# kmkolasinski/tfrecords-reader

Measured on AMD Instinct MI355X. Metric: GiB/s + examples/s device-resident TFRecord->Feature decode, 1/2/4/8 GPU, higher is better.
Workload: dtype u8; 1 GPU; C4 directory (configs[4]) of 256 files, C1-shaped (int64 label + 12 B bytes_list id) records, 524288 +-50 % per file (default_rng(1000+f)), spec CRC-32C; this rank's LPT share (256 files) resident in HBM; records_per_gpu=134295581, framed_bytes_per_gpu=7906235019, parallelism=file-sharded x1 (LPT by bytes, no collective on the data path), batches_per_gpu=4, batch_bytes_max=1976558779, streams=2, tpl_groups_missed=0

## Files before the change

### include/tfrg.h

```cpp
#ifndef TFRG_H
#define TFRG_H
#include <stdint.h>
#include "tfrg_status.h"

#ifdef __cplusplus
extern "C" {
#endif

#define TFRG_ABI_VERSION 1

#define TFRG_E_ARG (-1)
#define TFRG_E_HIP (-2)
#define TFRG_E_NOMEM (-3)
#define TFRG_E_IO (-4)
#define TFRG_E_LIMIT (-5)

#define TFRG_FLAG_PAYLOAD_ONLY 1u
#define TFRG_FLAG_SPEC_VARINT 2u
#define TFRG_FLAG_NO_CRC 4u
#define TFRG_FLAG_STRICT_CRC 8u
#define TFRG_FLAG_MATERIALIZE_BYTES 16u

int tfrg_abi_version(void);
const char* tfrg_status_exception(int status);
// ... 30 lines not shown
int tfrg_ctx_set_value_caps(tfrg_ctx* ctx, uint64_t int64_values, uint64_t float_values, uint64_t bytes_values);
int tfrg_ctx_device_bytes(tfrg_ctx* ctx, uint64_t* bytes, uint64_t* hint_reruns);
int tfrg_ctx_set_wave_stage(tfrg_ctx* ctx, uint32_t nbytes);
int tfrg_ctx_set_index_chunk(tfrg_ctx* ctx, uint32_t bytes);

#define TFRG_TPL_MAX 32
#define TFRG_TPL_MAX_PAYLOAD 240
#define TFRG_TPL_MAX_ENTRIES 16
#define TFRG_TPL_MAX_SLOTS 16
#define TFRG_TPL_SAMPLE 4096
int tfrg_learn_templates(tfrg_ctx* ctx, const uint8_t* h_bytes, uint64_t nbytes, const uint64_t* h_start,
                         const uint64_t* h_end, uint32_t n, uint32_t flags);
int tfrg_template_count(tfrg_ctx* ctx);
int tfrg_template_frames(tfrg_ctx* ctx);
int tfrg_template_words(tfrg_ctx* ctx, uint32_t* out, uint64_t cap, uint32_t* window_words);
int tfrg_learn_templates_host(uint32_t n_keys, const uint8_t* key_blob, const uint64_t* key_offsets,
                              const uint32_t* key_flags, uint32_t n_slots, const uint32_t* slot_key,
                              const uint8_t* slot_kind, const uint8_t* h_bytes, uint64_t nbytes,
                              const uint64_t* h_start, const uint64_t* h_end, uint32_t n, uint32_t flags,
                              uint32_t* out, uint64_t cap, uint32_t* window_words);
int tfrg_ctx_set_templates(tfrg_ctx* ctx, int on);

int tfrg_ctx_set_profiling(tfrg_ctx* ctx, int on);
int tfrg_profile_last(tfrg_ctx* ctx, float* ms, const char** names, int cap);

int tfrg_set_schema(tfrg_ctx* ctx, uint32_t n_keys, const uint8_t* key_blob, const uint64_t* key_offsets,
                    const uint32_t* key_flags, uint32_t n_slots, const uint32_t* slot_key,
                    const uint8_t* slot_kind);

typedef struct tfrg_host_ctx tfrg_host_ctx;
typedef struct tfrg_host_record {
  int32_t status;
  uint32_t n_entries;
  int64_t aux;
  const uint32_t* key_off;
  const uint32_t* key_len;
  const uint8_t* kind;
  const uint32_t* val_off;
  const uint32_t* val_cnt;
  const int64_t* i64;
  const uint32_t* f32;
  const uint32_t* b_off;
  const uint32_t* b_len;
} tfrg_host_record;
int tfrg_host_ctx_create(tfrg_host_ctx** out);
int tfrg_host_ctx_destroy(tfrg_host_ctx* ctx);
int tfrg_host_decode(tfrg_host_ctx* ctx, const uint8_t* payload, uint64_t len, uint32_t flags, tfrg_host_record* out);

int tfrg_decode_device(tfrg_ctx* ctx, const uint8_t* d_bytes, uint64_t nbytes, const uint64_t* d_start,
                       const uint64_t* d_end, uint32_t n, uint32_t flags, void* stream);
int tfrg_decode_device32(tfrg_ctx* ctx, const uint8_t* d_bytes, uint64_t nbytes, const uint32_t* d_start32,
                         const uint32_t* d_end32, uint32_t first_start, uint32_t n, uint32_t flags, void* stream);
int tfrg_decode_host(tfrg_ctx* ctx, const uint8_t* h_bytes, uint64_t nbytes, const uint64_t* h_start,
                     const uint64_t* h_end, uint32_t n, uint32_t flags, void* stream);

#define TFRG_INDEX_FB_ROUNDS 1u
#define TFRG_INDEX_FB_SEEK 2u
typedef struct tfrg_index_info {
  uint64_t n_records;
  uint32_t fallback;
  uint32_t tiled;
  uint32_t first_start;
  uint32_t n_chunks, repaired_chunks, repair_rounds;
} tfrg_index_info;
int tfrg_index_device(tfrg_ctx* ctx, const uint8_t* d_bytes, uint64_t nbytes, const uint64_t* piece_sizes,
                      uint32_t n_pieces, uint64_t* d_start, uint64_t* d_end, uint32_t* d_end32, uint64_t cap,
                      uint64_t* piece_records, void* stream, tfrg_index_info* info);

typedef struct tfrg_info {
  uint32_t n_records;
  uint32_t n_slots;
  uint32_t n_errors;
  uint32_t first_error;
  uint32_t n_miss_records;
  uint32_t n_miss_entries;
  uint32_t n_big;
  uint32_t scan_timeout;
  uint64_t kind_totals[4];
  uint64_t nbytes;
  uint64_t bytes_data_len;
  uint32_t tpl_groups_missed;
  uint32_t implicit_cols;
  uint64_t placed_slots;
} tfrg_info;

int tfrg_result_info(tfrg_ctx* ctx, tfrg_info* info);

typedef struct tfrg_columns {
  int32_t* status;
  int64_t* aux;
  uint8_t* verdict;
  uint16_t* order;
  uint32_t* row_splits;
  uint64_t* slot_base;
  int64_t* i64;
  uint32_t* f32;
  uint32_t* bytes_off;
  uint32_t* bytes_len;
  uint32_t* miss;
  uint8_t* bytes_data;
  uint64_t* bytes_offsets;
} tfrg_columns;

int tfrg_result_device(tfrg_ctx* ctx, tfrg_columns* cols);
int tfrg_result_fetch(tfrg_ctx* ctx, const tfrg_columns* host);

#define TFRG_DENSE_I64 0
#define TFRG_DENSE_I32 1
#define TFRG_DENSE_F32 2
#define TFRG_DENSE_U8 3
#define TFRG_DENSE_MAX_SPECS 64
#define TFRG_DENSE_MAX_WIDTH 4096
typedef struct tfrg_dense_spec {
  uint32_t slot;
  uint32_t dtype;
  uint32_t width;
  uint32_t reserved;
  uint64_t fill;
  void* out;
  int32_t* lengths;
} tfrg_dense_spec;
int tfrg_result_dense(tfrg_ctx* ctx, const tfrg_dense_spec* specs, uint32_t n_specs, uint32_t* d_stats,
                      void* consumer_stream);

#define TFRG_ROWS_I32 0
#define TFRG_ROWS_I64 1
int tfrg_result_dense_rows(tfrg_ctx* ctx, const tfrg_dense_spec* specs, uint32_t n_specs, const void* d_rows,
                           uint32_t rows_dtype, uint32_t m, int64_t row0, uint32_t* d_stats, uint32_t* d_skipped,
                           void* consumer_stream);

#define TFRG_RAGGED_MAX_SPECS 64
typedef struct tfrg_ragged_spec {
  uint32_t slot;
  uint32_t dtype;
  uint32_t max_len;
  uint32_t reserved;
  uint64_t cap;
  void* values;
  int64_t* offsets;
} tfrg_ragged_spec;
int tfrg_result_ragged_rows(tfrg_ctx* ctx, const tfrg_ragged_spec* specs, uint32_t n_specs,
                            const void* d_rows, uint32_t rows_dtype, uint32_t m, int64_t row0,
                            uint64_t* d_totals, uint32_t* d_stats, void* consumer_stream);
int tfrg_ctx_set_ragged_tile(tfrg_ctx* ctx, uint32_t rows);

#define TFRG_SEL_MAX_TERMS 32
#define TFRG_SEL_VALUE 0
#define TFRG_SEL_ANY 1
#define TFRG_SEL_COUNT 2
#define TFRG_SEL_BYTES_LEN 3
#define TFRG_SEL_STATUS 4
#define TFRG_SEL_EQ 0
#define TFRG_SEL_NE 1
#define TFRG_SEL_LT 2
#define TFRG_SEL_LE 3
#define TFRG_SEL_GT 4
#define TFRG_SEL_GE 5
typedef struct tfrg_select_term {
  uint32_t slot;
  uint32_t subject;
  uint32_t op;
  uint32_t group;
  uint32_t index;
  uint32_t reserved;
  uint64_t operand;
} tfrg_select_term;
#define TFRG_SEL_APPEND 1u
// ... 28 lines not shown
```

### tfrecords-reader_amd/csrc/tfrg_capi.cpp

```cpp
#include <hip/hip_runtime.h>
#include <stdlib.h>
#include <string.h>

#include <algorithm>
#include <map>
#include <numeric>
#include <string>
#include <unordered_map>
#include <vector>

#include "../../include/tfrg.h"
#include "crc32c.h"
#include "tfrg_dense.h"
#include "tfrg_ragged.h"
#include "tfrg_select.h"
#include "tfrg_frame.h"
#include "tfrg_internal.h"
#include "tfrg_learn.h"

namespace tfrg {
void set_error(const std::string& s);

#define HIP_TRY(expr)                                                              \
  do {                                                                             \
// ... 36 lines not shown

}

using namespace tfrg;

struct Offsets {
  const uint64_t* s64 = nullptr;
  const uint64_t* e64 = nullptr;
  const uint32_t* s32 = nullptr;
  const uint32_t* e32 = nullptr;
  uint32_t first = 0;
  uint32_t mode = kOffU64;
};

struct tfrg_ctx {
  int device = 0;
  hipStream_t own_stream = nullptr;
  hipStream_t last_stream = nullptr;
  uint32_t lane_max = 2048;
  uint32_t wave_stage = 0xffffffffu;
  uint64_t record_bound = 0;
  uint64_t call_bound = 0;
  int num_cus = 256;
  uint32_t cu_lds = 65536;
  int tpl_stage = 1;
  uint32_t tpl_gpw = 0;
  DBuf crc_tab, consts;
  DBuf ht, key_hash, key_off, key_blob, key_slot, slot_kind, key_w, krec;
  uint32_t n_keys = 0, n_slots = 0, ht_mask = 0;
  DBuf in_bytes, in_start, in_end;
  DBuf status, aux, verdict, order, count, loc, rs, slot_base, totals, kind_totals;
  DBuf ident;
  size_t ident_n = 0;
  DBuf i64, f32, b_off, b_len, big_list, slow_list, miss, info, tsum, crc_rec, crc_base, crc_part;
  DBuf dq, dq_cnt;
  DBuf lmask, rlist;
  DBuf bdata, boff64, blb, bbig;
  bool materialized = false;
  bool tsum_dirty = true;
  uint32_t info_slot = 0;
  bool info_clean = false;
  uint32_t n = 0;
  uint64_t cap_hint = 0;
  hipEvent_t order_ev = nullptr;
  hipEvent_t consumer_ev[2] = {nullptr, nullptr};
  int dense_nt = 0;
  uint64_t nbytes = 0;
  uint64_t cap_i64 = 0, cap_f32 = 0, cap_b = 0;
  bool have_result = false;
  bool rs_complete = false;
  std::unordered_map<std::string, uint32_t> key_id;
  std::vector<int32_t> key_slot_h;
  DBuf tpl;
  uint32_t n_tpl = 0;
  uint32_t tpl_w = 0;
  size_t tpl_img_off = 0;
  uint32_t tpl_img_words = 0;
  uint32_t tpl_tab_words = 0;
  std::vector<uint32_t> tpl_h;
  bool tpl_learned = false;
  bool tpl_full = false;
  uint32_t tpl_frames = 0;
  bool tpl_on = true;
  std::vector<uint8_t> slot_kind_h;
  DBuf spec;
  std::vector<uint32_t> spec_h;
  bool have_spec = false;
  bool spec_on = true;
  bool profiling = false;
  bool have_events = false;
  hipEvent_t ev[kNumStages + 1] = {};
  uint64_t hint_i64 = 0, hint_f32 = 0, hint_b = 0;
  bool hinted = false;
  bool no_hints = false;
  uint64_t hint_reruns = 0;
  bool optimistic_on = true;
  bool walk_beside = true;
  uint32_t walk_blocks = 0;
  bool no_quiet = false;
  bool opt_pending = false;
  bool ord_const = false;
  bool len_const = false;
  std::vector<uint32_t> const_len;
  uint32_t last_implicit = 0;
  bool last_aux_zero = false;
  uint32_t* info_pin = nullptr;
  bool cols_complete = false;
  bool mat_pending = false;
  struct LastCall {
    const uint8_t* d_bytes;
    uint64_t nbytes;
    uint64_t cap_in;
    uint64_t bound;
    uint32_t n, flags;
    hipStream_t st;
  } last{};
  Offsets last_off{};
  uint32_t index_chunk = kIndexChunkDefault;
  DBuf fr_tab, fr_dev;
  uint32_t ragged_tile = kRaggedTileDefault;
  DBuf rg_tsum;
  uint32_t select_tile = kSelTileDefault;
  DBuf sel_buf;
  void* fr_pin = nullptr;
  size_t fr_pin_cap = 0;
  uint32_t poison[4] = {0xffffffffu, 0xffffffffu, 0xffffffffu, 0xffffffffu};
};

extern "C" {

int tfrg_ctx_create(int device, tfrg_ctx** out) {
  *out = nullptr;
  int ndev = 0;
  HIP_TRY(hipGetDeviceCount(&ndev));
  if (device < 0 || device >= ndev) {
    set_error("bad device index");
    return TFRG_E_ARG;
  }
  HIP_TRY(hipSetDevice(device));
  tfrg_ctx* c = new tfrg_ctx();
  c->device = device;
  if (const char* e = getenv("TFRG_TEMPLATES")) c->tpl_on = atoi(e) != 0;
  if (const char* e = getenv("TFRG_SPEC")) c->spec_on = atoi(e) != 0;
  if (const char* e = getenv("TFRG_TPL_STAGE")) c->tpl_stage = atoi(e);
  if (const char* e = getenv("TFRG_TPL_GPW")) {
    const int v = atoi(e);
    if (v == 2 || v == 4 || v == 8) c->tpl_gpw = (uint32_t)v;
  }
  if (const char* e = getenv("TFRG_OPTIMISTIC")) c->optimistic_on = atoi(e) != 0;
  if (const char* e = getenv("TFRG_WALK_BESIDE")) c->walk_beside = atoi(e) != 0;
  if (const char* e = getenv("TFRG_WALK_BLOCKS")) c->walk_blocks = (uint32_t)atoi(e);
  if (const char* e = getenv("TFRG_DENSE_NT")) c->dense_nt = atoi(e) != 0;
  if (const char* e = getenv("TFRG_DEBUG_POISON_LOC")) {
    char* q = const_cast<char*>(e);
    for (int i = 0; i < 4 && *q; ++i) {
      c->poison[i] = (uint32_t)strtoul(q, &q, 10);
      while (*q == ',' || *q == ' ') ++q;
    }
  }
  hipDeviceProp_t prop;
  if (hipGetDeviceProperties(&prop, device) == hipSuccess) {
    c->num_cus = prop.multiProcessorCount;
    if (prop.maxSharedMemoryPerMultiProcessor) c->cu_lds = (uint32_t)prop.maxSharedMemoryPerMultiProcessor;
  }
  if (hipStreamCreateWithFlags(&c->own_stream, hipStreamNonBlocking) != hipSuccess) {
    delete c;
    set_error("hipStreamCreate failed");
    return TFRG_E_HIP;
  }
  if (hipHostMalloc(reinterpret_cast<void**>(&c->info_pin), (kInfoCount + 8) * 4) != hipSuccess) {
    (void)hipStreamDestroy(c->own_stream);
    delete c;
    set_error("hipHostMalloc failed");
    return TFRG_E_NOMEM;
  }
  std::vector<uint32_t> tab(kCrcTabWords), cst(128);
  CrcTables T;
  crc_make_tables(&T);
  memcpy(tab.data(), T.t, 4096);
  uint32_t M[4][256];
  crc_make_mul_tables(gf_xpow8(1024), M);
  memcpy(tab.data() + 1024, M, 4096);
  memcpy(tab.data() + 2048, T.t, 8192);
  memcpy(tab.data() + 4096, T.t, 16384);
  for (int e = 0; e < 256; ++e)
    for (int col = 0; col < 47; ++col) tab[8192 + e * 64 + col] = T.t[(col + 1) & 15][e];
  crc_make_mul_tables(gf_xpow8(2048), M);
  memcpy(tab.data() + 24576, M, 4096);
  crc_make_mul_tables(gf_xpow8(4096), M);
  memcpy(tab.data() + 25600, M, 4096);
  for (int k = 0; k < 24; ++k) {
    crc_make_mul_tables(gf_xpow8(1024ull << k), M);
    memcpy(tab.data() + 26624 + k * 1024, M, 4096);
  }
  for (int l = 0; l < 64; ++l) cst[l] = gf_xpow8(16ull * l);
  for (int z = 0; z < 16; ++z) cst[64 + z] = gf_xpow8_inv((uint64_t)z);
  for (int k = 0; k < 32; ++k) cst[96 + k] = gf_xpow8(1024ull << k);
  if (c->crc_tab.ensure(tab.size() * 4) != hipSuccess || c->consts.ensure(cst.size() * 4) != hipSuccess ||
      hipMemcpy(c->crc_tab.p, tab.data(), tab.size() * 4, hipMemcpyHostToDevice) != hipSuccess ||
      hipMemcpy(c->consts.p, cst.data(), cst.size() * 4, hipMemcpyHostToDevice) != hipSuccess) {
    set_error("constant upload failed");
    tfrg_ctx_destroy(c);
    return TFRG_E_HIP;
  }
  *out = c;
  return 0;
}

int tfrg_ctx_destroy(tfrg_ctx* c) {
  if (!c) return 0;
  (void)hipSetDevice(c->device);
  if (c->last_stream) (void)hipStreamSynchronize(c->last_stream);
  DBuf* all[] = {&c->crc_tab, &c->consts, &c->ht, &c->key_hash, &c->key_off, &c->key_blob, &c->key_slot,
                 &c->slot_kind, &c->key_w, &c->krec, &c->in_bytes, &c->in_start, &c->in_end, &c->status, &c->aux, &c->verdict,
                 &c->order, &c->count, &c->loc, &c->rs, &c->ident, &c->slot_base, &c->totals, &c->kind_totals, &c->i64,
                 &c->f32, &c->b_off, &c->b_len, &c->big_list, &c->slow_list, &c->miss, &c->info, &c->tsum,
                 &c->bdata, &c->boff64, &c->blb, &c->bbig, &c->crc_rec, &c->crc_base, &c->crc_part, &c->tpl, &c->spec,
                 &c->dq, &c->dq_cnt, &c->lmask, &c->rlist, &c->fr_tab, &c->fr_dev, &c->rg_tsum, &c->sel_buf};
  for (DBuf* b : all) b->release();
  if (c->order_ev) (void)hipEventDestroy(c->order_ev);
  for (hipEvent_t e : c->consumer_ev)
    if (e) (void)hipEventDestroy(e);
  if (c->have_events)
    for (auto& e : c->ev) (void)hipEventDestroy(e);
  if (c->own_stream) (void)hipStreamDestroy(c->own_stream);
  if (c->info_pin) (void)hipHostFree(c->info_pin);
  if (c->fr_pin) (void)hipHostFree(c->fr_pin);
  delete c;
  return 0;
}

int tfrg_ctx_set_lane_max(tfrg_ctx* c, uint32_t lane_max) {
// ... 167 lines not shown
}

static void key_words(const uint8_t* p, uint64_t n, uint32_t* w0, uint32_t* w1) {
  uint32_t a = 0, b = 0;
  for (uint64_t i = 0; i < (n < 4 ? n : 4); ++i) a |= (uint32_t)p[i] << (8 * i);
  if (n > 4)
    for (uint64_t i = 0; i < 4; ++i) b |= (uint32_t)p[n - 4 + i] << (8 * i);
  *w0 = a;
  *w1 = b;
}

int tfrg_set_schema(tfrg_ctx* c, uint32_t n_keys, const uint8_t* key_blob, const uint64_t* key_offsets,
                    const uint32_t* key_flags, uint32_t n_slots, const uint32_t* slot_key, const uint8_t* slot_kind) {
  if (!c) return TFRG_E_ARG;
  HIP_TRY(hipSetDevice(c->device));
  if (c->last_stream) HIP_TRY(hipStreamSynchronize(c->last_stream));
  c->have_result = false;
  c->n_keys = c->n_slots = 0;
  c->ht_mask = 0;
  uint32_t hsz = 16;
  while (hsz < 2 * n_keys + 2) hsz <<= 1;
  std::vector<uint32_t> ht(hsz, 0), hash(n_keys ? n_keys : 1), off(n_keys + 1), kw(2ull * (n_keys ? n_keys : 1));
  std::vector<int32_t> ks(4ull * (n_keys ? n_keys : 1), -1);
  const uint64_t blob_len = n_keys ? key_offsets[n_keys] : 0;
  for (uint32_t k = 0; k < n_keys; ++k) {
    if (key_offsets[k + 1] < key_offsets[k] || key_offsets[k + 1] > 0xffffffffull) {
      set_error("bad key offsets");
      return TFRG_E_ARG;
    }
    off[k] = (uint32_t)key_offsets[k];
    const uint64_t kl = key_offsets[k + 1] - key_offsets[k];
    key_words(key_blob + key_offsets[k], kl, &kw[2ull * k], &kw[2ull * k + 1]);
    hash[k] = key_hash_words((uint32_t)kl, kw[2ull * k], kw[2ull * k + 1]);
    ks[4ull * k] = (int32_t)(key_flags ? (key_flags[k] & 1u) : 0u);
    uint32_t j = hash[k] & (hsz - 1);
    while (ht[j]) j = (j + 1) & (hsz - 1);
    ht[j] = k + 1;
  }
  off[n_keys] = (uint32_t)blob_len;
  for (uint32_t s = 0; s < n_slots; ++s) {
    if (slot_key[s] >= n_keys || slot_kind[s] < 1 || slot_kind[s] > 3) {
      set_error("bad slot");
      return TFRG_E_ARG;
    }
    ks[4ull * slot_key[s] + slot_kind[s]] = (int32_t)s;
  }
  if (c->ht.ensure(hsz * 4) || c->key_hash.ensure(hash.size() * 4) || c->key_off.ensure(off.size() * 4) ||
      c->key_blob.ensure(blob_len + 16) || c->key_slot.ensure(ks.size() * 4) || c->slot_kind.ensure(n_slots + 16) ||
      c->key_w.ensure(kw.size() * 4)) {
    set_error("schema allocation failed");
    return TFRG_E_NOMEM;
  }
  HIP_TRY(hipMemcpy(c->ht.p, ht.data(), hsz * 4, hipMemcpyHostToDevice));
  HIP_TRY(hipMemcpy(c->key_hash.p, hash.data(), hash.size() * 4, hipMemcpyHostToDevice));
  HIP_TRY(hipMemcpy(c->key_off.p, off.data(), off.size() * 4, hipMemcpyHostToDevice));
  if (blob_len) HIP_TRY(hipMemcpy(c->key_blob.p, key_blob, blob_len, hipMemcpyHostToDevice));
  HIP_TRY(hipMemcpy(c->key_slot.p, ks.data(), ks.size() * 4, hipMemcpyHostToDevice));
  HIP_TRY(hipMemcpy(c->key_w.p, kw.data(), kw.size() * 4, hipMemcpyHostToDevice));
  std::vector<uint32_t> kr((size_t)kKrWords * (n_keys ? n_keys : 1), 0);
  for (uint32_t k = 0; k < n_keys; ++k) {
    uint32_t* r = &kr[(size_t)kKrWords * k];
    r[kKrHash] = hash[k];
    r[kKrLen] = (uint32_t)(key_offsets[k + 1] - key_offsets[k]);
    r[kKrW0] = kw[2ull * k];
    r[kKrW1] = kw[2ull * k + 1];
    for (int kind = 1; kind <= 3; ++kind) r[kKrSlot1 + kind - 1] = (uint32_t)ks[4ull * k + kind];
    r[kKrFlags] = (uint32_t)ks[4ull * k];
  }
  if (c->krec.ensure(kr.size() * 4)) {
    set_error("schema allocation failed");
    return TFRG_E_NOMEM;
  }
  HIP_TRY(hipMemcpy(c->krec.p, kr.data(), kr.size() * 4, hipMemcpyHostToDevice));
  if (n_slots) HIP_TRY(hipMemcpy(c->slot_kind.p, slot_kind, n_slots, hipMemcpyHostToDevice));
  c->n_keys = n_keys;
  c->n_slots = n_slots;
  c->ht_mask = hsz - 1;
  c->key_id.clear();
  for (uint32_t k = 0; k < n_keys; ++k)
    c->key_id.emplace(std::string((const char*)key_blob + key_offsets[k], key_offsets[k + 1] - key_offsets[k]), k);
  c->key_slot_h = ks;
  c->slot_kind_h.assign(slot_kind, slot_kind + n_slots);
  c->n_tpl = 0;
  c->tpl_learned = false;
  c->have_spec = false;
  return 0;
}

static DevSchema schema_view(const tfrg_ctx* c) {
  DevSchema s;
  s.n_keys = c->n_keys;
  s.n_slots = c->n_slots;
  s.ht_mask = c->ht_mask;
  s.ht = c->ht.as<uint32_t>();
  s.key_hash = c->key_hash.as<uint32_t>();
  s.key_off = c->key_off.as<uint32_t>();
  s.key_blob = c->key_blob.as<uint8_t>();
  s.key_slot = c->key_slot.as<int32_t>();
  s.slot_kind = c->slot_kind.as<uint8_t>();
  s.key_w = c->key_w.as<uint32_t>();
  s.krec = c->krec.as<uint32_t>();
  s.tpl = c->tpl.as<uint32_t>();
  s.tpl_img = s.tpl + c->tpl_img_off;
  s.tpl_img_words = c->tpl_img_words;
  s.tpl_tab_words = c->tpl_tab_words;
  s.n_tpl = c->tpl_on ? c->n_tpl : 0u;
  s.tpl_w = c->tpl_w;
  s.spec = c->spec_on && c->have_spec ? c->spec.as<uint32_t>() : nullptr;
  return s;
}

extern "C" int tfrg_learn_templates(tfrg_ctx* c, const uint8_t* h_bytes, uint64_t nbytes, const uint64_t* h_start,
                                    const uint64_t* h_end, uint32_t n, uint32_t flags) {
  if (!c || (n && (!h_bytes || !h_start || !h_end))) return TFRG_E_ARG;
  c->tpl_learned = true;
  c->n_tpl = 0;
  c->tpl_frames = 0;
  c->have_spec = false;
  if (!c->n_keys) return 0;
  const TplSchema sch{c->key_id, c->key_slot_h, c->slot_kind_h};
  Learned L;
  const uint32_t nt = learn_shapes(&sch, c->n_slots, h_bytes, nbytes, h_start, h_end, n, flags, L);
  if (!nt && !(L.have_spec = learn_single_slots(&sch, c->n_slots, h_bytes, nbytes, h_start, h_end, n, flags, L.spec)))
    return 0;
  const size_t spec_bytes = (size_t)c->n_slots * 4;
  HIP_TRY(hipSetDevice(c->device));
  if (c->last_stream) HIP_TRY(hipStreamSynchronize(c->last_stream));
  if ((nt && c->tpl.ensure((L.w.size() + L.img.size() + L.ptab.size()) * 4)) ||
      (L.have_spec && c->spec.ensure(spec_bytes))) {
    set_error("template allocation failed");
    return TFRG_E_NOMEM;
  }
  if (nt) {
    uint32_t* const d = c->tpl.as<uint32_t>();
    HIP_TRY(hipMemcpy(d, L.w.data(), L.w.size() * 4, hipMemcpyHostToDevice));
    HIP_TRY(hipMemcpy(d + L.w.size(), L.img.data(), L.img.size() * 4, hipMemcpyHostToDevice));
    if (!L.ptab.empty())
      HIP_TRY(hipMemcpy(d + L.w.size() + L.img.size(), L.ptab.data(), L.ptab.size() * 4, hipMemcpyHostToDevice));
    c->tpl_img_off = L.w.size();
    c->tpl_img_words = (uint32_t)L.img.size();
    c->tpl_tab_words = (uint32_t)L.ptab.size();
    c->n_tpl = nt;
    c->tpl_w = L.W;
    c->tpl_h = L.w;
    c->tpl_full = L.full;
    c->tpl_frames = L.frames;
    c->ord_const = L.ord_const;
    c->len_const = L.len_const;
    c->const_len = L.const_len;
  }
  if (L.have_spec) HIP_TRY(hipMemcpy(c->spec.p, L.spec.data(), spec_bytes, hipMemcpyHostToDevice));
  c->spec_h = L.spec;
  c->have_spec = L.have_spec;
  return (int)nt;
}

extern "C" int tfrg_template_count(tfrg_ctx* c) { return c ? (int)c->n_tpl : TFRG_E_ARG; }

extern "C" int tfrg_template_frames(tfrg_ctx* c) { return c ? (int)(c->n_tpl ? c->tpl_frames : 0u) : TFRG_E_ARG; }

extern "C" int tfrg_template_words(tfrg_ctx* c, uint32_t* out, uint64_t cap, uint32_t* window_words) {
  if (!c) return TFRG_E_ARG;
  if (window_words) *window_words = c->tpl_w;
  const uint64_t nw = (uint64_t)c->n_tpl * kLtWords;
  if (out) memcpy(out, c->tpl_h.data(), (nw < cap ? nw : cap) * 4);
  return (int)c->n_tpl;
}

extern "C" int tfrg_ctx_set_templates(tfrg_ctx* c, int on) {
  if (!c) return TFRG_E_ARG;
  c->tpl_on = on != 0;
  return 0;
}

static int decode_device_any(tfrg_ctx* c, const uint8_t* d_bytes, uint64_t nbytes, const Offsets& off, uint32_t n,
                             uint32_t flags, void* stream);

int tfrg_decode_device(tfrg_ctx* c, const uint8_t* d_bytes, uint64_t nbytes, const uint64_t* d_start,
                       const uint64_t* d_end, uint32_t n, uint32_t flags, void* stream) {
  Offsets off;
  off.s64 = d_start;
  off.e64 = d_end;
  return decode_device_any(c, d_bytes, nbytes, off, n, flags, stream);
}

int tfrg_decode_device32(tfrg_ctx* c, const uint8_t* d_bytes, uint64_t nbytes, const uint32_t* d_start32,
                         const uint32_t* d_end32, uint32_t first_start, uint32_t n, uint32_t flags, void* stream) {
  if (n && !d_end32) return TFRG_E_ARG;
  Offsets off;
  off.s32 = d_start32;
  off.e32 = d_end32;
  off.first = first_start;
  off.mode = d_start32 ? kOffU32 : kOffEnds;
  return decode_device_any(c, d_bytes, nbytes, off, n, flags, stream);
}

static hipError_t launch_materialize_last(tfrg_ctx* c, const uint8_t* d_bytes, uint64_t nbytes, uint64_t cap_in,
                                          uint64_t cap_b, hipStream_t st) {
  uint32_t* const info = c->info.as<uint32_t>() + c->info_slot * kInfoCount;
  DevBytes d;
  d.in = d_bytes;
  d.in_readable = (nbytes + 15) & ~15ull;
  d.b_off = c->b_off.as<uint32_t>();
  d.b_len = c->b_len.as<uint32_t>();
  d.kind_totals = c->kind_totals.as<uint64_t>();
  d.offsets = c->boff64.as<uint64_t>();
  d.offsets_cap = cap_b;
  d.data = c->bdata.as<uint8_t>();
  d.data_cap = cap_in + 16;
  d.lb = c->blb.as<uint64_t>();
  d.ticket = info + kInfoBytesTicket;
  d.big_count = info + kInfoBytesBig;
  d.big_list = c->bbig.as<uint32_t>();
  d.overflow = info + kInfoOverflow;
  return launch_materialize(d, c->num_cus, st);
}

static int decode_device_any(tfrg_ctx* c, const uint8_t* d_bytes, uint64_t nbytes, const Offsets& off, uint32_t n,
                             uint32_t flags, void* stream) {
  if (!c) return TFRG_E_ARG;
  if (nbytes >= (1ull << 32)) {
    set_error("batch larger than 4 GiB: split it");
    return TFRG_E_LIMIT;
  }
  if (c->n_keys == 0) {
    uint64_t z = 0;
    int st = tfrg_set_schema(c, 0, nullptr, &z, nullptr, 0, nullptr, nullptr);
    if (st) return st;
  }
  HIP_TRY(hipSetDevice(c->device));
  c->have_result = false;
  hipStream_t st = stream ? (hipStream_t)stream : c->own_stream;
// ... 63 lines not shown
                    c->bbig.cap < cap_b * 4;
    if (g2 && c->last_stream) HIP_TRY(hipStreamSynchronize(c->last_stream));
    if (c->bdata.ensure(cap_in + 16) || c->boff64.ensure((cap_b + 1) * 8) || c->blb.ensure(lb_words * 8) ||
        c->bbig.ensure(cap_b * 4)) {
      set_error("device allocation failed (materialized bytes)");
      return TFRG_E_NOMEM;
    }
    HIP_TRY(hipMemsetAsync(c->blb.p, 0, lb_words * 8, st));
    if (!n) HIP_TRY(hipMemsetAsync(c->boff64.p, 0, 8, st));
  }
  if (!S || !n) HIP_TRY(hipMemsetAsync(c->kind_totals.p, 0, 32, st));

  DevBatch b;
  b.bytes = d_bytes;
  b.nbytes = nbytes;
  b.start = off.s64;
  b.end = off.e64;
  b.start32 = off.s32;
  b.end32 = off.e32;
  b.first = off.first;
  b.omode = off.mode;
  b.n = n;
  b.flags = flags;
  DevOut o;
  o.status = c->status.as<int32_t>();
  o.aux = c->aux.as<int64_t>();
  o.verdict = c->verdict.as<uint8_t>();
  o.order = c->order.as<uint16_t>();
  o.count = c->count.as<uint32_t>();
  o.loc = c->loc.as<uint2>();
  o.rs = c->rs.as<uint32_t>();
  o.slot_base = c->slot_base.as<uint64_t>();
  o.totals = c->totals.as<uint32_t>();
  o.kind_totals = c->kind_totals.as<uint64_t>();
  o.i64 = c->i64.as<int64_t>();
  o.f32 = c->f32.as<uint32_t>();
  o.b_off = c->b_off.as<uint32_t>();
  o.b_len = c->b_len.as<uint32_t>();
  o.cap_i64 = cap_i64;
  o.cap_f32 = cap_f32;
  o.cap_b = cap_b;
  o.big_list = c->big_list.as<uint32_t>();
  o.miss = c->miss.as<uint32_t>();
  o.miss_cap = kMissCap;
  o.info = info_cur;
  o.info_next = c->info.as<uint32_t>() + (islot ^ 1u) * kInfoCount;
  o.tsum = c->tsum.as<uint32_t>();
  o.tile_stride = tile_stride;
  o.spine_lb = reinterpret_cast<uint64_t*>(o.tsum + (size_t)S * tile_stride);
  o.n_chunks = n_chunks;
  o.irr = o.tsum + (size_t)S * tile_stride + 2ull * S * n_chunks;
  o.slow_list = c->slow_list.as<uint32_t>();
  o.crc_rec = c->crc_rec.as<uint32_t>();
  o.crc_base = c->crc_base.as<uint64_t>();
  o.crc_part = c->crc_part.as<uint64_t>();
  o.lmask = c->lmask.as<uint64_t>();
  o.rlist = c->rlist.as<uint32_t>();
  LaunchCfg cfg;
  cfg.num_cus = c->num_cus;
  cfg.tpl_cu_lds = c->tpl_stage ? c->cu_lds : 0u;
  cfg.tpl_stage_any = c->tpl_stage == 2;
  cfg.tpl_gpw = c->tpl_gpw;
  cfg.lean = c->tpl_on && c->n_tpl;
  cfg.tpl_full = cfg.lean && c->tpl_full;
  cfg.tpl_unchecked = cfg.lean && (c->tpl_frames & 2u) != 0;
  cfg.spec_h = c->spec_h.empty() ? nullptr : c->spec_h.data();
  const uint64_t lane_blocks = (n + 255) / 256;
  const uint64_t lane_cap = (uint64_t)c->num_cus * 8;
  cfg.lane_grid = (int)(lane_blocks < 1 ? 1 : (lane_blocks < lane_cap ? lane_blocks : lane_cap));
  const uint64_t wave_cap = (uint64_t)c->num_cus * 4;
  const uint64_t wave_blocks = (n + 3) / 4;
  cfg.wave_grid = (int)(wave_blocks < 1 ? 1 : (wave_blocks < wave_cap ? wave_blocks : wave_cap));
  cfg.lane_max = c->lane_max;
  cfg.wave_stage = c->wave_stage;
  memcpy(cfg.poison, c->poison, sizeof(cfg.poison));
  cfg.optimistic = c->optimistic_on && !c->no_quiet && c->poison[0] == 0xffffffffu;
  cfg.walk_beside = c->walk_beside;
  cfg.walk_blocks = c->walk_blocks;
  cfg.ran_optimistic = false;
  cfg.ran_quiet_big = false;
  cfg.ord_const = c->ord_const;
  cfg.len_const = c->len_const && !mat;
  cfg.implicit = 0;
  const uint64_t bound = c->call_bound ? c->call_bound : c->record_bound;
  c->call_bound = 0;
  c->last = tfrg_ctx::LastCall{d_bytes, nbytes, cap_in, bound, n, flags, st};
  c->last_off = off;
  o.dq = nullptr;
  o.dq_cnt = nullptr;
  o.dq_blocks = 0;
  cfg.body_count = false;
  if (n && (bound == 0 || bound > c->lane_max)) {
    uint64_t blocks = nbytes >> 18;
    blocks = blocks < 16 ? 16 : (blocks > (1u << 16) ? (1u << 16) : blocks);
    const size_t qb = (size_t)blocks * 64u * kDeferK * 16u, cb = (size_t)blocks * 64u;
    if ((c->dq.cap < qb || c->dq_cnt.cap < cb) && c->last_stream) HIP_TRY(hipStreamSynchronize(c->last_stream));
    if (c->dq.ensure(qb) || c->dq_cnt.ensure(cb)) {
      set_error("device allocation failed (deferred bodies)");
      return TFRG_E_NOMEM;
    }
    o.dq = c->dq.as<uint4>();
    o.dq_cnt = c->dq_cnt.as<uint8_t>();
    o.dq_blocks = (uint32_t)blocks;
    cfg.body_count = true;
  }
  if (n) {
    hipEvent_t* ev = nullptr;
    if (c->profiling) {
      if (!c->have_events) {
        for (auto& e : c->ev) HIP_TRY(hipEventCreate(&e));
        c->have_events = true;
      }
      ev = c->ev;
    }
    hipError_t e = launch_decode(b, schema_view(c), o, cfg, c->crc_tab.as<uint32_t>(), c->consts.as<uint32_t>(), st, ev);
    if (e == hipSuccess && mat && S && !cfg.ran_optimistic) {
      e = launch_materialize_last(c, d_bytes, nbytes, cap_in, cap_b, st);
    } else if (e == hipSuccess && mat && !S) {
      e = hipMemsetAsync(c->boff64.p, 0, 8, st);
    }
    if (ev && e == hipSuccess) e = hipEventRecord(ev[kNumStages], st);
    if (e != hipSuccess) {
      c->tsum_dirty = true;
      set_error(std::string("kernel launch: ") + hipGetErrorString(e));
      return TFRG_E_HIP;
    }
  }
  c->info_clean = n != 0;
  c->n = n;
  c->nbytes = nbytes;
  c->cap_i64 = cap_i64;
  c->cap_f32 = cap_f32;
  c->cap_b = cap_b;
  c->last_stream = st;
  c->materialized = mat;
  c->have_result = true;
  c->rs_complete = false;
  c->opt_pending = n != 0 && cfg.ran_optimistic;
  if (n != 0 && cfg.ran_quiet_big) c->tsum_dirty = true;
  c->mat_pending = c->opt_pending && mat && S;
  c->last_implicit = n != 0 ? cfg.implicit : 0u;
  c->last_aux_zero = n != 0 && cfg.ran_optimistic && !cfg.ran_quiet_big && !(cfg.implicit & TFRG_IMPLICIT_STATUS);
  c->cols_complete = false;
  return 0;
}

int tfrg_decode_host(tfrg_ctx* c, const uint8_t* h_bytes, uint64_t nbytes, const uint64_t* h_start,
                     const uint64_t* h_end, uint32_t n, uint32_t flags, void* stream) {
  if (!c) return TFRG_E_ARG;
  HIP_TRY(hipSetDevice(c->device));
  hipStream_t st = stream ? (hipStream_t)stream : c->own_stream;
  const uint64_t pad = ((nbytes + 15) & ~15ull) + 16;
  if (c->last_stream) HIP_TRY(hipStreamSynchronize(c->last_stream));
  if (c->in_bytes.ensure(pad) || c->in_start.ensure((uint64_t)(n ? n : 1) * 8) ||
      c->in_end.ensure((uint64_t)(n ? n : 1) * 8)) {
    set_error("staging allocation failed");
    return TFRG_E_NOMEM;
  }
  if (nbytes) HIP_TRY(hipMemcpyAsync(c->in_bytes.p, h_bytes, nbytes, hipMemcpyHostToDevice, st));
  HIP_TRY(hipMemsetAsync(c->in_bytes.as<uint8_t>() + nbytes, 0, pad - nbytes, st));
  if (n) {
    HIP_TRY(hipMemcpyAsync(c->in_start.p, h_start, (size_t)n * 8, hipMemcpyHostToDevice, st));
    HIP_TRY(hipMemcpyAsync(c->in_end.p, h_end, (size_t)n * 8, hipMemcpyHostToDevice, st));
  }
  uint64_t total = 0, widest = 0;
  for (uint32_t i = 0; i < n; ++i) {
    const uint64_t a = h_start[i], b = h_end[i] < nbytes ? h_end[i] : nbytes;
    if (b > a) total += b - a;
    if (h_end[i] > a && h_end[i] - a > widest) widest = h_end[i] - a;
  }
  if (!c->tpl_learned && c->n_keys && c->tpl_on) {
    const int t = tfrg_learn_templates(c, h_bytes, nbytes, h_start, h_end, n, flags);
    if (t < 0) return t;
  }
  c->cap_hint = total;
  c->call_bound = widest ? widest : 1;
  return tfrg_decode_device(c, c->in_bytes.as<uint8_t>(), nbytes, c->in_start.as<uint64_t>(),
                            c->in_end.as<uint64_t>(), n, flags, st);
}

static int finish_decode(tfrg_ctx* c, uint32_t* h, uint64_t* kt) {
  bool widened = false;
  for (;;) {
    HIP_TRY(hipMemcpyAsync(c->info_pin, c->info.as<uint32_t>() + c->info_slot * kInfoCount, kInfoCount * 4,
                           hipMemcpyDeviceToHost, c->last_stream));
    HIP_TRY(hipMemcpyAsync(c->info_pin + kInfoCount, c->kind_totals.p, 32, hipMemcpyDeviceToHost, c->last_stream));
    HIP_TRY(hipStreamSynchronize(c->last_stream));
    memcpy(h, c->info_pin, kInfoCount * 4);
    memcpy(kt, c->info_pin + kInfoCount, 32);
    const bool full = c->opt_pending && h[kInfoResid] != 0;
    const bool widen = h[kInfoOverflow] && c->hinted && !widened;
    if (!full && !widen) {
      if (!c->mat_pending) break;
      c->mat_pending = false;
      const tfrg_ctx::LastCall& L = c->last;
      HIP_TRY(launch_materialize_last(c, L.d_bytes, L.nbytes, L.cap_in, c->cap_b, c->last_stream));
      continue;
    }
    const tfrg_ctx::LastCall L = c->last;
    c->no_quiet = true;
    c->no_hints = widen;
    c->cap_hint = L.cap_in;
    c->call_bound = L.bound;
    c->tsum_dirty = true;
    const int rc = decode_device_any(c, L.d_bytes, L.nbytes, c->last_off, L.n, L.flags, L.st);
    c->no_quiet = false;
    c->no_hints = false;
    if (rc) return rc;
    widened |= widen;
    ++c->hint_reruns;
  }
  c->opt_pending = false;
  c->hinted = false;
  return 0;
}

static int overflow_status(const uint32_t* h) {
  if (!h[kInfoOverflow]) return 0;
  set_error("value columns overflowed their capacity (overlapping ranges in a device batch): decode "
            "the ranges from host memory (tfrg_decode_host) or split the batch");
  return TFRG_E_LIMIT;
}

static int confirm_pending(tfrg_ctx* c) {
  if (!c->opt_pending && !c->hinted) return 0;
  HIP_TRY(hipSetDevice(c->device));
  uint32_t h[kInfoCount];
  uint64_t kt[4];
  const int rc = finish_decode(c, h, kt);
  return rc ? rc : overflow_status(h);
}

int tfrg_result_info(tfrg_ctx* c, tfrg_info* info) {
  if (!c || !c->have_result) return TFRG_E_ARG;
  HIP_TRY(hipSetDevice(c->device));
  uint32_t h[kInfoCount] = {0};
  uint64_t kt[4] = {0, 0, 0, 0};
  const int rc = finish_decode(c, h, kt);
  if (rc) return rc;
  uint64_t blen = 0;
  if (c->materialized && !h[kInfoOverflow]) {
    const uint64_t nb = c->n ? kt[TFRG_KIND_BYTES] : 0;
    HIP_TRY(hipMemcpy(&blen, c->boff64.as<uint64_t>() + nb, 8, hipMemcpyDeviceToHost));
  }
  memset(info, 0, sizeof(*info));
  info->n_records = c->n;
  info->n_slots = c->n_slots;
  info->n_errors = h[kInfoErrors];
  info->first_error = ~h[kInfoFirstError];
  info->n_miss_records = h[kInfoMissRecords];
  info->n_miss_entries = h[kInfoMissEntries];
  info->n_big = h[kInfoBigRecs];
  info->scan_timeout = h[kInfoScanTimeout];
  for (int k = 0; k < 4; ++k) info->kind_totals[k] = kt[k];
  info->nbytes = c->nbytes;
  info->bytes_data_len = blen;
  info->tpl_groups_missed = h[kInfoResid];
  info->placed_slots = ((uint64_t)h[kInfoPlacedHi] << 32) | h[kInfoPlacedLo];
  info->implicit_cols = c->last_implicit;
  return overflow_status(h);
}

static std::vector<std::pair<uint64_t, uint32_t>> implicit_len_runs(const tfrg_ctx* c) {
  std::vector<std::pair<uint64_t, uint32_t>> out;
  uint64_t base = 0;
  for (uint32_t k = 0; k < c->n_slots; ++k) {
    if ((c->slot_kind_h[k] & 3u) != TFRG_KIND_BYTES) continue;
    out.push_back({base, k < c->const_len.size() ? c->const_len[k] : 0u});
    base += c->n;
  }
  return out;
}

int tfrg_result_device(tfrg_ctx* c, tfrg_columns* d) {
  if (!c || !c->have_result) return TFRG_E_ARG;
  if (const int rc = confirm_pending(c)) return rc;
  if (!c->rs_complete && c->n_slots && c->n) {
    HIP_TRY(hipSetDevice(c->device));
    HIP_TRY(launch_fill_placed_rows(c->rs.as<uint32_t>(), c->info.as<uint32_t>() + c->info_slot * kInfoCount,
                                    c->n_slots, c->n, c->last_stream));
  }
  c->rs_complete = true;
  if ((c->last_implicit || c->last_aux_zero) && !c->cols_complete) {
    HIP_TRY(hipSetDevice(c->device));
    const size_t n = c->n;
    if (c->last_aux_zero) HIP_TRY(hipMemsetAsync(c->aux.p, 0, n * 8, c->last_stream));
    if (c->last_implicit & TFRG_IMPLICIT_STATUS) {
      HIP_TRY(hipMemsetAsync(c->status.p, 0, n * 4, c->last_stream));
      HIP_TRY(hipMemsetAsync(c->aux.p, 0, n * 8, c->last_stream));
      HIP_TRY(hipMemsetAsync(c->verdict.p, (int)(TFRG_V_LEN_MATCH | TFRG_V_LEN_CRC | TFRG_V_DATA_CRC), n, c->last_stream));
    }
    if (c->last_implicit & TFRG_IMPLICIT_ORDER)
      for (uint32_t k = 0; k < c->n_slots; ++k)
        HIP_TRY(hipMemsetD16Async(reinterpret_cast<hipDeviceptr_t>(c->order.as<uint16_t>() + (size_t)k * n),
                                  (unsigned short)(c->tpl_h[kLtSlot + 3 * k] >> 16), n, c->last_stream));
    if (c->last_implicit & TFRG_IMPLICIT_BYTES_LEN)
      for (const auto& [base, len] : implicit_len_runs(c))
        HIP_TRY(hipMemsetD32Async(reinterpret_cast<hipDeviceptr_t>(c->b_len.as<uint32_t>() + base), (int)len, n,
                                  c->last_stream));
  }
  c->cols_complete = true;
  d->status = c->status.as<int32_t>();
  d->aux = c->aux.as<int64_t>();
  d->verdict = c->verdict.as<uint8_t>();
  d->order = c->order.as<uint16_t>();
  d->row_splits = c->rs.as<uint32_t>();
  d->slot_base = c->slot_base.as<uint64_t>();
  d->i64 = c->i64.as<int64_t>();
  d->f32 = c->f32.as<uint32_t>();
  d->bytes_off = c->b_off.as<uint32_t>();
  d->bytes_len = c->b_len.as<uint32_t>();
  d->miss = c->miss.as<uint32_t>();
  d->bytes_data = c->materialized ? c->bdata.as<uint8_t>() : nullptr;
  d->bytes_offsets = c->materialized ? c->boff64.as<uint64_t>() : nullptr;
  return 0;
}

extern "C++" {
template <class Bad>
static int check_result(const tfrg_ctx* c, const Bad& bad) {
  if (!c) return bad("no context");
  if (!c->have_result) return bad("no result (decode first)");
  return 0;
}
template <class Bad>
static int check_specs(const tfrg_ctx* c, const void* specs, uint32_t n_specs, uint32_t max_specs, const Bad& bad) {
  if (const int rc = check_result(c, bad)) return rc;
  if (!specs || n_specs == 0 || n_specs > max_specs) return bad("n_specs must be 1.." + std::to_string(max_specs));
  return 0;
}
template <class Bad>
static int check_slot_dtype(const tfrg_ctx* c, const std::string& at, uint32_t slot, uint32_t dtype, const Bad& bad) {
  if (slot >= c->n_slots) return bad(at + "slot " + std::to_string(slot) + " >= n_slots");
  const uint32_t kind = c->slot_kind_h[slot] & 3u;
  const bool fits = (kind == TFRG_KIND_INT64 && (dtype == TFRG_DENSE_I64 || dtype == TFRG_DENSE_I32)) ||
                    (kind == TFRG_KIND_FLOAT && dtype == TFRG_DENSE_F32) ||
                    (kind == TFRG_KIND_BYTES && dtype == TFRG_DENSE_U8);
  if (!fits) return bad(at + "dtype " + std::to_string(dtype) + " does not fit the slot's kind " + std::to_string(kind));
  return 0;
}
template <class Bad>
static int check_rows_dtype(const void* d_rows, uint32_t rows_dtype, bool required, const Bad& bad) {
  if ((required || d_rows) && rows_dtype != TFRG_ROWS_I32 && rows_dtype != TFRG_ROWS_I64)
    return bad("rows_dtype must be TFRG_ROWS_I32 or TFRG_ROWS_I64, not " + std::to_string(rows_dtype));
  return 0;
}
template <class Bad>
static int check_rows_m(const void* d_rows, uint32_t m, bool required, const Bad& bad) {
  if (m >= 0x80000000u) return bad("m must be below 2^31");
  if (required && m && !d_rows) return bad("d_rows is NULL");
  return 0;
}

template <class T>
static const T* view_col(const tfrg_ctx* c, const DBuf& b) {
  return static_cast<const T*>(b.p ? b.p : c->slot_base.p);
}
template <class Args>
static void fill_columns(const tfrg_ctx* c, Args& a) {
  a.rs = c->rs.as<uint32_t>();
  a.slot_base = c->slot_base.as<uint64_t>();
  a.i64 = view_col<int64_t>(c, c->i64);
  a.f32 = view_col<uint32_t>(c, c->f32);
  a.b_len = view_col<uint32_t>(c, c->b_len);
  if (c->materialized) a.b_off64 = view_col<uint64_t>(c, c->boff64);
  a.info = c->info.as<uint32_t>() + c->info_slot * kInfoCount;
  a.n = c->n;
}
template <class Args>
static void fill_bytes_source(const tfrg_ctx* c, Args& a) {
  a.b_off = view_col<uint32_t>(c, c->b_off);
  a.in = c->materialized ? c->bdata.as<uint8_t>() : c->last.d_bytes;
  const uint64_t bound = c->materialized ? (uint64_t)c->bdata.cap & ~15ull : (c->last.nbytes + 15ull) & ~15ull;
  a.in_bound = a.in ? (uint32_t)std::min<uint64_t>(bound, 0xfffffff0ull) : 0;
}
}

static_assert(kDenseNoLen == kRaggedNoLen && kRaggedNoLen == kSelNoLen, "one const_len lookup serves all three");
static uint32_t const_len_of(const tfrg_ctx* c, uint32_t slot, bool reads_len) {
  if (!reads_len || !(c->last_implicit & TFRG_IMPLICIT_BYTES_LEN)) return kDenseNoLen;
  return slot < c->const_len.size() ? c->const_len[slot] : 0u;
}

static int fence_open(tfrg_ctx* c, void* consumer_stream, hipStream_t* st, hipStream_t* cs) {
  *st = c->last_stream;
  *cs = consumer_stream ? static_cast<hipStream_t>(consumer_stream) : *st;
  if (*cs == *st) return 0;
  for (hipEvent_t& e : c->consumer_ev)
    if (!e) HIP_TRY(hipEventCreateWithFlags(&e, hipEventDisableTiming));
  HIP_TRY(hipEventRecord(c->consumer_ev[0], *cs));
  HIP_TRY(hipStreamWaitEvent(*st, c->consumer_ev[0], 0));
  return 0;
}
static int fence_close(tfrg_ctx* c, hipStream_t st, hipStream_t cs) {
  if (cs == st) return 0;
  HIP_TRY(hipEventRecord(c->consumer_ev[1], st));
  HIP_TRY(hipStreamWaitEvent(cs, c->consumer_ev[1], 0));
  return 0;
}

struct DenseRows {
  const void* d_rows = nullptr;
  uint32_t dtype = 0, m = 0;
  int64_t row0 = 0;
  uint32_t* d_skipped = nullptr;
};

static int result_dense(const char* fn, bool by_rows, tfrg_ctx* c, const tfrg_dense_spec* specs, uint32_t n_specs,
                        const DenseRows& rows, uint32_t* d_stats, void* consumer_stream) {
  auto bad = [fn](const std::string& why) {
    set_error(std::string(fn) + ": " + why);
    return TFRG_E_ARG;
  };
  if (const int rc = check_specs(c, specs, n_specs, TFRG_DENSE_MAX_SPECS, bad)) return rc;
  static_assert(TFRG_DENSE_MAX_SPECS == kDenseMaxSpecs && TFRG_DENSE_MAX_WIDTH == kDenseMaxWidth &&
                    TFRG_DENSE_I64 == kDenseI64 && TFRG_DENSE_I32 == kDenseI32 && TFRG_DENSE_F32 == kDenseF32 &&
                    TFRG_DENSE_U8 == kDenseU8,
                "tfrg.h mirrors tfrg_dense.h");
  for (uint32_t i = 0; i < n_specs; ++i) {
    const tfrg_dense_spec& s = specs[i];
    const std::string at = "spec " + std::to_string(i) + ": ";
    if (const int rc = check_slot_dtype(c, at, s.slot, s.dtype, bad)) return rc;
    if (s.width == 0 || s.width > TFRG_DENSE_MAX_WIDTH)
      return bad(at + "width must be 1.." + std::to_string(TFRG_DENSE_MAX_WIDTH));
    if (!s.out) return bad(at + "out is NULL");
    if (s.reserved) return bad(at + "reserved must be 0");
  }
  if (by_rows) {
    if (const int rc = check_rows_dtype(rows.d_rows, rows.dtype, true, bad)) return rc;
    if (const int rc = check_rows_m(rows.d_rows, rows.m, true, bad)) return rc;
  }
  if (!by_rows && c->n == 0) return 0;
  HIP_TRY(hipSetDevice(c->device));
  if (const int rc = confirm_pending(c)) return rc;
  const uint32_t out_rows = by_rows ? rows.m : c->n;
  DenseArgs a{};
  if (by_rows) {
    a.rows = rows.d_rows;
    a.rows64 = rows.dtype == TFRG_ROWS_I64;
    a.m = rows.m;
    a.row0 = rows.row0;
    a.skipped = rows.d_skipped;
  }
  fill_columns(c, a);
  fill_bytes_source(c, a);
  a.stats = d_stats;
  a.n_specs = n_specs;
  a.nt = (uint32_t)c->dense_nt;
  const uint64_t cap = std::max<uint64_t>(1, (uint64_t)c->num_cus * 16u / n_specs);
  uint32_t blocks = 0;
  for (uint32_t i = 0; i < n_specs; ++i) {
    const tfrg_dense_spec& s = specs[i];
    DenseSpec& d = a.sp[i];
    d.out = s.out;
    d.lengths = s.lengths;
    d.fill = s.fill;
    d.slot = s.slot;
    d.dtype = s.dtype;
    d.width = s.width;
    d.const_len = const_len_of(c, s.slot, s.dtype == TFRG_DENSE_U8);
    const uint64_t isz = s.dtype == TFRG_DENSE_I64 ? 8 : s.dtype == TFRG_DENSE_U8 ? 1 : 4;
    const uint64_t total = (uint64_t)out_rows * s.width * isz;
    const uint64_t work = ((uintptr_t)s.out & 15u) ? total / isz : (total >> 4) + 16;
    d.blk0 = blocks;
    d.nblk = (uint32_t)std::min<uint64_t>(cap, (work + kDenseChunk - 1) / kDenseChunk);
    blocks += d.nblk;
  }
  hipStream_t st, cs;
  if (const int rc = fence_open(c, consumer_stream, &st, &cs)) return rc;
  const bool one_memset = by_rows && c->n && d_stats && rows.d_skipped == d_stats + 4 * (size_t)n_specs;
  if (d_stats) HIP_TRY(hipMemsetAsync(d_stats, 0, (size_t)n_specs * (one_memset ? 20 : 16), st));
  if (by_rows && rows.d_skipped && !one_memset)
    HIP_TRY(hipMemsetD32Async(reinterpret_cast<hipDeviceptr_t>(rows.d_skipped), c->n ? 0 : (int)rows.m, n_specs, st));
  if (out_rows && c->n) HIP_TRY(launch_dense(a, blocks, st));
  return fence_close(c, st, cs);
}

int tfrg_result_dense(tfrg_ctx* c, const tfrg_dense_spec* specs, uint32_t n_specs, uint32_t* d_stats,
                      void* consumer_stream) {
  return result_dense("tfrg_result_dense", false, c, specs, n_specs, DenseRows{}, d_stats, consumer_stream);
}

int tfrg_result_dense_rows(tfrg_ctx* c, const tfrg_dense_spec* specs, uint32_t n_specs, const void* d_rows,
                           uint32_t rows_dtype, uint32_t m, int64_t row0, uint32_t* d_stats, uint32_t* d_skipped,
                           void* consumer_stream) {
  DenseRows rows;
  rows.d_rows = d_rows;
  rows.dtype = rows_dtype;
  rows.m = m;
  rows.row0 = row0;
  rows.d_skipped = d_skipped;
  return result_dense("tfrg_result_dense_rows", true, c, specs, n_specs, rows, d_stats, consumer_stream);
}

int tfrg_result_ragged_rows(tfrg_ctx* c, const tfrg_ragged_spec* specs, uint32_t n_specs, const void* d_rows,
                            uint32_t rows_dtype, uint32_t m, int64_t row0, uint64_t* d_totals, uint32_t* d_stats,
                            void* consumer_stream) {
  auto bad = [](const std::string& why) {
    set_error("tfrg_result_ragged_rows: " + why);
    return TFRG_E_ARG;
  };
  if (const int rc = check_specs(c, specs, n_specs, TFRG_RAGGED_MAX_SPECS, bad)) return rc;
  static_assert(TFRG_RAGGED_MAX_SPECS == kRaggedMaxSpecs, "tfrg.h mirrors tfrg_ragged.h");
  bool any_values = false;
  for (uint32_t i = 0; i < n_specs; ++i) {
    const tfrg_ragged_spec& s = specs[i];
    const std::string at = "spec " + std::to_string(i) + ": ";
    if (const int rc = check_slot_dtype(c, at, s.slot, s.dtype, bad)) return rc;
    if (!s.offsets) return bad(at + "offsets is NULL");
    if (s.reserved) return bad(at + "reserved must be 0");
    const uintptr_t isz = s.dtype == TFRG_DENSE_I64 ? 8 : s.dtype == TFRG_DENSE_U8 ? 1 : 4;
    if (((uintptr_t)s.values & (isz - 1)) || ((uintptr_t)s.offsets & 7u))
      return bad(at + "values and offsets must be aligned to their element size");
    any_values |= s.values != nullptr && s.cap != 0;
  }
  if (const int rc = check_rows_dtype(d_rows, rows_dtype, false, bad)) return rc;
  if (const int rc = check_rows_m(d_rows, m, false, bad)) return rc;
  const uint32_t tile = c->ragged_tile;
  const uint64_t tiles = ((uint64_t)m + tile - 1) / tile;
  uint64_t split = 1;
  if (any_values && tiles) {
    const uint64_t want = (uint64_t)std::max(c->num_cus, 1) * 4u, have = tiles * n_specs;
    split = std::min<uint64_t>(kRaggedMaxSplit, std::max<uint64_t>(1, (want + have - 1) / have));
  }
  if (tiles * n_specs * split > 0x7fffffffull) return bad("too many tiles for one launch: raise the ragged tile");
  HIP_TRY(hipSetDevice(c->device));
  if (const int rc = confirm_pending(c)) return rc;
  const bool run = m && c->n;
  if (run) HIP_TRY(c->rg_tsum.ensure((size_t)(tiles * n_specs) * 8));
  hipStream_t st, cs;
  if (const int rc = fence_open(c, consumer_stream, &st, &cs)) return rc;
  if (d_stats) HIP_TRY(hipMemsetAsync(d_stats, 0, (size_t)n_specs * 16, st));
  if (run) {
    RaggedArgs a{};
    fill_columns(c, a);
    fill_bytes_source(c, a);
    a.stats = d_stats;
    a.totals = d_totals;
    a.tsum = c->rg_tsum.as<uint64_t>();
    a.rows = d_rows;
    a.rows64 = rows_dtype == TFRG_ROWS_I64;
    a.row0 = row0;
    a.m = m;
    a.n_specs = n_specs;
    a.tile = tile;
    a.tiles = (uint32_t)tiles;
    a.split = (uint32_t)split;
    for (uint32_t i = 0; i < n_specs; ++i) {
      const tfrg_ragged_spec& s = specs[i];
      RaggedSpec& d = a.sp[i];
      d.values = s.values;
      d.offsets = s.offsets;
      d.cap = s.cap;
      d.slot = s.slot;
      d.dtype = s.dtype;
      d.max_len = s.max_len;
      d.const_len = const_len_of(c, s.slot, s.dtype == TFRG_DENSE_U8);
    }
    HIP_TRY(launch_ragged(a, st));
  } else {
    for (uint32_t i = 0; i < n_specs; ++i) {
      HIP_TRY(hipMemsetAsync(specs[i].offsets, 0, ((size_t)m + 1) * 8, st));
      if (d_stats && m)
        HIP_TRY(hipMemsetD32Async(reinterpret_cast<hipDeviceptr_t>(d_stats + 4 * (size_t)i + 3), (int)m, 1, st));
    }
    if (d_totals) HIP_TRY(hipMemsetAsync(d_totals, 0, (size_t)n_specs * 8, st));
  }
  return fence_close(c, st, cs);
}

int tfrg_result_select_rows(tfrg_ctx* c, const tfrg_select_term* terms, uint32_t n_terms, const void* d_rows,
                            uint32_t rows_dtype, uint32_t m, int64_t row0, void* d_out, uint32_t out_dtype,
                            uint64_t cap, uint64_t* d_count, uint32_t* d_stats, uint32_t flags, void* consumer_stream) {
  auto bad = [](const std::string& why) {
    set_error("tfrg_result_select_rows: " + why);
    return TFRG_E_ARG;
  };
  if (const int rc = check_result(c, bad)) return rc;
  static_assert(TFRG_SEL_MAX_TERMS == kSelMaxTerms && TFRG_SEL_VALUE == kSelValue && TFRG_SEL_ANY == kSelAny &&
                    TFRG_SEL_COUNT == kSelCount && TFRG_SEL_BYTES_LEN == kSelBytesLen &&
                    TFRG_SEL_STATUS == kSelStatus && TFRG_SEL_EQ == kSelEq && TFRG_SEL_GE == kSelGe &&
                    sizeof(tfrg_select_term) == 32,
                "tfrg.h mirrors tfrg_select.h");
  if (n_terms > TFRG_SEL_MAX_TERMS) return bad("n_terms must be at most " + std::to_string(TFRG_SEL_MAX_TERMS));
  if (n_terms && !terms) return bad("terms is NULL");
  for (uint32_t i = 0; i < n_terms; ++i) {
    const tfrg_select_term& t = terms[i];
    const std::string at = "term " + std::to_string(i) + ": ";
    if (t.slot >= c->n_slots) return bad(at + "slot " + std::to_string(t.slot) + " >= n_slots");
    if (t.subject > TFRG_SEL_STATUS) return bad(at + "unknown subject " + std::to_string(t.subject));
    if (t.op > TFRG_SEL_GE) return bad(at + "unknown op " + std::to_string(t.op));
    if (t.group >= 32) return bad(at + "group must be below 32");
    const uint32_t kind = c->slot_kind_h[t.slot] & 3u;
    const bool list = t.subject == TFRG_SEL_VALUE || t.subject == TFRG_SEL_ANY;
    if ((list && kind != TFRG_KIND_INT64 && kind != TFRG_KIND_FLOAT) ||
        (t.subject == TFRG_SEL_BYTES_LEN && kind != TFRG_KIND_BYTES) || (t.subject == TFRG_SEL_STATUS && t.slot != 0))
      return bad(at + "subject " + std::to_string(t.subject) + " does not fit slot " + std::to_string(t.slot) +
                 " of kind " + std::to_string(kind));
    if (t.index && t.subject != TFRG_SEL_VALUE) return bad(at + "index must be 0 outside TFRG_SEL_VALUE");
    if (t.reserved) return bad(at + "reserved must be 0");
    if (list && kind == TFRG_KIND_FLOAT && (t.operand >> 32)) return bad(at + "a float operand has its high 32 bits set");
  }
  if (const int rc = check_rows_dtype(d_rows, rows_dtype, false, bad)) return rc;
  if (out_dtype != TFRG_ROWS_I32 && out_dtype != TFRG_ROWS_I64)
    return bad("out_dtype must be TFRG_ROWS_I32 or TFRG_ROWS_I64, not " + std::to_string(out_dtype));
  if (const int rc = check_rows_m(d_rows, m, false, bad)) return rc;
  if (!d_count) return bad("d_count is NULL");
  if (((uintptr_t)d_count & 7u) || ((uintptr_t)d_out & (out_dtype == TFRG_ROWS_I64 ? 7u : 3u)))
    return bad("d_out and d_count must be aligned to their element size");
  if (out_dtype == TFRG_ROWS_I32 && c->n &&
      (row0 < (int64_t)INT32_MIN || row0 > (int64_t)INT32_MAX - ((int64_t)c->n - 1)))
    return bad("rows [row0, row0 + n) do not fit an int32 output");
  if (flags & ~TFRG_SEL_APPEND) return bad("unknown flag bits");
  const bool append = (flags & TFRG_SEL_APPEND) != 0;
  HIP_TRY(hipSetDevice(c->device));
  if (const int rc = confirm_pending(c)) return rc;
  const uint32_t tile = c->select_tile;
  const uint64_t tiles = ((uint64_t)m + tile - 1) / tile, nwords = ((uint64_t)m + 63) / 64;
  const bool run = m && c->n;
  if (run) HIP_TRY(c->sel_buf.ensure((size_t)(nwords + tiles) * 8));
  hipStream_t st, cs;
  if (const int rc = fence_open(c, consumer_stream, &st, &cs)) return rc;
  if (d_stats) HIP_TRY(hipMemsetAsync(d_stats, 0, 8, st));
  if (run) {
    SelectArgs a{};
    fill_columns(c, a);
    a.status = (c->last_implicit & TFRG_IMPLICIT_STATUS) ? nullptr : c->status.as<int32_t>();
    a.stats = d_stats;
    a.count = d_count;
    a.words = c->sel_buf.as<uint64_t>();
    a.tsum = a.words + nwords;
    a.rows = d_rows;
    a.out = d_out;
    a.cap = d_out ? cap : 0;
    a.row0 = row0;
    a.m = m;
    a.rows64 = rows_dtype == TFRG_ROWS_I64;
    a.out64 = out_dtype == TFRG_ROWS_I64;
    a.n_terms = n_terms;
    a.tile = tile;
    a.tiles = (uint32_t)tiles;
    a.append = append;
    for (uint32_t i = 0; i < n_terms; ++i) {
      const tfrg_select_term& t = terms[i];
      SelTerm& d = a.term[i];
      d.slot = t.slot;
      d.subject = t.subject;
      d.op = t.op;
      d.group = t.group;
      d.index = t.index;
      d.rhs = (int64_t)t.operand;
      const bool list = t.subject == TFRG_SEL_VALUE || t.subject == TFRG_SEL_ANY;
      if (list && (c->slot_kind_h[t.slot] & 3u) == TFRG_KIND_FLOAT) {
        d.is_float = 1;
        d.rhs_nan = sel_float_nan((uint32_t)t.operand);
        d.rhs = d.rhs_nan ? 0 : sel_float_key((uint32_t)t.operand);
      }
      d.const_len = const_len_of(c, t.slot, t.subject == TFRG_SEL_BYTES_LEN);
      a.all_groups |= 1u << t.group;
    }
    HIP_TRY(launch_select(a, st));
  } else {
    if (!append) HIP_TRY(hipMemsetAsync(d_count, 0, 8, st));
    if (d_stats && m) HIP_TRY(hipMemsetD32Async(reinterpret_cast<hipDeviceptr_t>(d_stats + 1), (int)m, 1, st));
  }
  return fence_close(c, st, cs);
}

int tfrg_result_fetch(tfrg_ctx* c, const tfrg_columns* h) {
  tfrg_info info;
  int rc = tfrg_result_info(c, &info);
  if (rc) return rc;
  const hipStream_t st = c->last_stream;
  const size_t n = c->n, S = c->n_slots;
  auto cp = [&](void* dst, const void* src, size_t bytes) -> hipError_t {
    if (!dst || !bytes) return hipSuccess;
    return hipMemcpyAsync(dst, src, bytes, hipMemcpyDeviceToHost, st);
  };
  if (info.implicit_cols & TFRG_IMPLICIT_STATUS) {
    if (h->status) memset(h->status, 0, n * 4);
    if (h->aux) memset(h->aux, 0, n * 8);
    if (h->verdict) memset(h->verdict, TFRG_V_LEN_MATCH | TFRG_V_LEN_CRC | TFRG_V_DATA_CRC, n);
  } else {
    HIP_TRY(cp(h->status, c->status.p, n * 4));
    if (c->last_aux_zero) {
      if (h->aux) memset(h->aux, 0, n * 8);
    } else {
      HIP_TRY(cp(h->aux, c->aux.p, n * 8));
    }
    HIP_TRY(cp(h->verdict, c->verdict.p, n));
  }
  if ((info.implicit_cols & TFRG_IMPLICIT_ORDER) && h->order) {
    for (size_t k = 0; k < S; ++k) std::fill_n(h->order + k * n, n, (uint16_t)(c->tpl_h[kLtSlot + 3 * k] >> 16));
  } else {
    HIP_TRY(cp(h->order, c->order.p, S * n * 2));
  }
  if (h->row_splits) {
    if (S && (info.placed_slots & (S >= 64 ? ~0ull : (1ull << S) - 1ull)) && c->ident_n < n + 1) {
      const size_t m = std::max<size_t>(n + 1, 2 * c->ident_n);
      std::vector<uint32_t> v(m);
      std::iota(v.begin(), v.end(), 0u);
      c->ident_n = 0;
      HIP_TRY(c->ident.ensure(m * 4));
      HIP_TRY(hipMemcpy(c->ident.p, v.data(), m * 4, hipMemcpyHostToDevice));
      c->ident_n = m;
    }
    for (size_t k = 0; k < S; ++k) {
      const bool pk = k < 64 && ((info.placed_slots >> k) & 1ull);
      HIP_TRY(cp(h->row_splits + k * (n + 1), pk ? c->ident.as<uint32_t>() : c->rs.as<uint32_t>() + k * (n + 1),
                 (n + 1) * 4));
    }
  }
  HIP_TRY(cp(h->slot_base, c->slot_base.p, S * 8));
  auto cl = [](uint64_t v, uint64_t cap) { return v < cap ? v : cap; };
  HIP_TRY(cp(h->i64, c->i64.p, cl(info.kind_totals[TFRG_KIND_INT64], c->cap_i64) * 8));
  HIP_TRY(cp(h->f32, c->f32.p, cl(info.kind_totals[TFRG_KIND_FLOAT], c->cap_f32) * 4));
  HIP_TRY(cp(h->bytes_off, c->b_off.p, cl(info.kind_totals[TFRG_KIND_BYTES], c->cap_b) * 4));
  if ((info.implicit_cols & TFRG_IMPLICIT_BYTES_LEN) && h->bytes_len) {
    for (const auto& [base, len] : implicit_len_runs(c)) std::fill_n(h->bytes_len + base, n, len);
  } else {
    HIP_TRY(cp(h->bytes_len, c->b_len.p, cl(info.kind_totals[TFRG_KIND_BYTES], c->cap_b) * 4));
  }
  if (c->materialized) {
    HIP_TRY(cp(h->bytes_data, c->bdata.p, info.bytes_data_len));
    HIP_TRY(cp(h->bytes_offsets, c->boff64.p, (info.kind_totals[TFRG_KIND_BYTES] + 1) * 8));
  }
  const size_t nm = info.n_miss_entries < kMissCap ? info.n_miss_entries : kMissCap;
  HIP_TRY(cp(h->miss, c->miss.p, nm * 16));
  HIP_TRY(hipStreamSynchronize(st));
  return 0;
}

}

int tfrg_stream_read(const void* d_bytes, uint64_t nbytes, uint32_t* d_sink, void* stream, int variant) {
  if (!d_bytes || !d_sink || (nbytes & 15u)) return TFRG_E_ARG;
  return tfrg::launch_stream_read(d_bytes, nbytes, d_sink, static_cast<hipStream_t>(stream), variant) == hipSuccess
             ? 0 : TFRG_E_HIP;
}

int tfrg_device_count(void) {
  int n = 0;
  if (hipGetDeviceCount(&n) != hipSuccess) return 0;
  return n;
}
```

### tfrecords-reader_amd/csrc/tfrg_decode.cpp

```cpp
#include <algorithm>

#include "../../include/tfrg_status.h"
#include "tfrg_internal.h"

namespace tfrg {

const char* const kStageNames[kNumStages] = {"k_tpl_lane",    "k_lane_count",  "k_body_count", "k_tail_count", "k_spine",
                                             "k_down_gather", "k_tail_gather", "k_bytes"};

static LeanArgs lean_args(const DevBatch& b, const DevSchema& sc, const DevOut& o, const LaunchCfg& cfg,
                          bool placing) {
  const bool nocrc = (b.flags & kFlagNoCrc) != 0;
  LeanArgs a{};
  a.n_tpl = sc.n_tpl;
  a.img_words = sc.tpl_img_words;
  a.tab_words = nocrc ? 0u : sc.tpl_tab_words;
  a.nocrc = nocrc ? 1u : 0u;
  a.strict = (b.flags & kFlagStrictCrc) ? 1u : 0u;
  a.uframes = cfg.tpl_unchecked ? 1u : 0u;
  a.cu_lds = cfg.tpl_cu_lds;
  a.stage_any = cfg.tpl_stage_any ? 1u : 0u;
  a.gpw_force = cfg.tpl_gpw;
  a.lane_max = cfg.lane_max;
  a.tsum = cfg.ran_optimistic ? nullptr : o.tsum;
  a.finish = cfg.ran_optimistic ? sc.slot_kind : nullptr;
  a.implicit = cfg.implicit;
  a.n_slots = sc.n_slots;
  a.tile_stride = o.tile_stride;
  const uint64_t n = b.n;
  for (uint32_t k = 0; k < sc.n_slots; ++k) {
    LeanTgt& t = a.tg[k];
    t.ord = o.order + k * n;
    t.cnt = o.count + k * n;
    t.loc = o.loc + k * n;
    t.rs = o.rs + k * (n + 1);
    const uint32_t sw = placing ? cfg.spec_h[k] : 0u;
    if (!sw) continue;
    const uint32_t kind = sw & 3u;
    const uint64_t base = n * ((sw >> 2) - 1u);
    const uint64_t cap = kind == TFRG_KIND_INT64 ? o.cap_i64 : kind == TFRG_KIND_FLOAT ? o.cap_f32 : o.cap_b;
    t.lim = cap > base ? (uint32_t)std::min<uint64_t>(cap - base, n) : 0u;
    t.kind = kind;
    if (kind == TFRG_KIND_INT64) t.v1 = o.i64 + base;
    else if (kind == TFRG_KIND_FLOAT) t.v1 = o.f32 + base;
    else t.v1 = o.b_off + base;
    t.v2 = o.b_len + base;
  }
  return a;
}

hipError_t launch_decode(const DevBatch& b, const DevSchema& sc, const DevOut& o, LaunchCfg& cfg,
                         const uint32_t* d_tab, const uint32_t* d_consts, hipStream_t st, hipEvent_t* ev) {
  auto mark = [&](int i) {
    if (ev) (void)hipEventRecord(ev[i], st);
  };
  auto mark_rest = [&](int from) {
    for (int i = from; i <= kStageMaterialize; ++i) mark(i);
    return hipGetLastError();
  };
  const uint32_t S = sc.n_slots, cus = (uint32_t)cfg.num_cus;
  const uint32_t n_tiles = (b.n + kTileRecs - 1) / kTileRecs;
  const bool fast_ok = schema_in_lds(sc);
  const int lane_mode = lane_count_mode(sc);
  DevSchema scx = sc;
  if (lane_mode != 0 || !fast_ok) scx.spec = nullptr;
  const bool lean = cfg.lean && sc.n_tpl && fast_ok && S <= kLeanMaxSlots && o.lmask && o.rlist &&
                    (sc.tpl_w == 16 || sc.tpl_w == 32 || sc.tpl_w == 64) &&
                    !(b.flags & kFlagPayloadOnly) && b.nbytes < 0xffffff00ull;
  const bool tpl_nocrc = (b.flags & kFlagNoCrc) != 0, tpl_strict = (b.flags & kFlagStrictCrc) != 0;
  const bool quiet = lean && cfg.tpl_full && !cfg.body_count;
  bool all_spec = scx.spec && cfg.spec_h && S <= 64;
  for (uint32_t k = 0; all_spec && k < S; ++k) all_spec = cfg.spec_h[k] != 0u;
  const bool quiet_tpl = cfg.optimistic && quiet && all_spec && S > 0 && !(tpl_strict && cfg.tpl_unchecked);
  const bool quiet_big = cfg.optimistic && !lean && all_spec && S > 0 && lane_mode == 0 && fast_ok &&
                         cfg.body_count && !tpl_strict && b.n > 0;
  cfg.ran_optimistic = quiet_tpl || quiet_big;
  cfg.ran_quiet_big = quiet_big;
  const bool walk_beside = quiet_big && cfg.walk_beside && tail_walk_fits(sc);
  cfg.implicit = lean && cfg.ran_optimistic ? (!tpl_nocrc && !cfg.tpl_unchecked ? TFRG_IMPLICIT_STATUS : 0u) |
                                                  (cfg.ord_const ? TFRG_IMPLICIT_ORDER : 0u) |
                                                  (cfg.len_const ? TFRG_IMPLICIT_BYTES_LEN : 0u)
                                            : 0u;
  DevOut ox = o;
  if (!lean) {
    ox.lmask = nullptr;
    ox.rlist = nullptr;
  }
  mark(kStageTplLane);
  if (lean) {
    const LeanArgs a = lean_args(b, sc, o, cfg, scx.spec && cfg.spec_h);
    const hipError_t e = launch_tpl_lane(b, ox, a, sc.tpl_img, sc.tpl_w, cfg.num_cus, st);
    if (e != hipSuccess) return e;
  }
  if (quiet_tpl) return mark_rest(kStageLaneCount);
  mark(kStageLaneCount);
  launch_lane_count(b, scx, ox, d_tab, cfg, walk_beside, lane_mode, std::min(cfg.lane_grid, quiet ? 64 : cfg.lane_grid), st);
  mark(kStageBodyCount);
  if (cfg.body_count && lane_mode != 0) launch_body_count(b, ox, cfg.num_cus, st);
  mark(kStageTailCount);
  const uint32_t tail_cap = std::max(8u, (uint32_t)(b.nbytes >> 16) + b.n / 4096u);
  launch_tail_count(b, scx, ox, d_tab, d_consts, cfg, quiet_big, walk_beside,
                    cfg.body_count ? tail_cap : std::min(tail_cap, 32u), st);
  if (quiet_big) return mark_rest(kStageSpine);
  if (cfg.poison[0] != 0xffffffffu && S > 0) launch_poison_loc(ox, b.n, S, cfg.poison, st);
  mark(kStageSpine);
  if (S > 0) launch_spine(ox, scx, n_tiles, b.n, st);
  mark(kStageDownGather);
  if (S > 0) {
    uint32_t resident = all_spec ? std::min(cus, std::max(8u, n_tiles / 4u)) : 8u * cus;
    if (all_spec && quiet) resident = std::min(resident, 32u);
    launch_down_gather(b, scx, ox, cfg, n_tiles, resident, st);
  }
  mark(kStageTailGather);
  if (S > 0) {
    int cap = (int)std::min<uint64_t>((uint64_t)cfg.wave_grid,
                                      std::max<uint64_t>(8u, std::max<uint64_t>(b.n / 1024u, b.nbytes >> 16)));
    if (quiet && all_spec) cap = std::min(cap, 32);
    launch_tail_gather(b, scx, ox, cfg, cap, st);
  }
  mark(kStageMaterialize);
  return hipGetLastError();
}

}
```

### tfrecords-reader_amd/csrc/tfrg_dense.h

```cpp
#pragma once
#include <stdint.h>
#include <hip/hip_runtime.h>

namespace tfrg {

constexpr uint32_t kDenseMaxSpecs = 64;
constexpr uint32_t kDenseMaxWidth = 4096;
enum DenseType : uint32_t { kDenseI64 = 0, kDenseI32 = 1, kDenseF32 = 2, kDenseU8 = 3 };
constexpr uint32_t kDenseNoLen = 0xffffffffu;

constexpr uint32_t kDenseChunk = 1024;

struct DenseSpec {
  void* out;
  int32_t* lengths;
  uint64_t fill;
  uint32_t slot;
  uint32_t dtype;
  uint32_t width;
  uint32_t const_len;
  uint32_t blk0;
  uint32_t nblk;
};

struct DenseArgs {
  const uint32_t* rs;
  const uint64_t* slot_base;
  const int64_t* i64;
  const uint32_t* f32;
  const uint32_t* b_off;
  const uint32_t* b_len;
  const uint64_t* b_off64;
  const uint8_t* in;
  const uint32_t* info;
  uint32_t* stats;
  const void* rows;
  uint32_t* skipped;
  int64_t row0;
  uint32_t m;
  uint32_t rows64;
  uint32_t in_bound;
  uint32_t n;
  uint32_t n_specs;
  uint32_t nt;
  DenseSpec sp[kDenseMaxSpecs];
};
static_assert(sizeof(DenseArgs) <= 4096, "k_dense's spec table travels as the kernel argument");

hipError_t launch_dense(const DenseArgs& a, uint32_t blocks, hipStream_t st);

}
```

### tfrecords-reader_amd/csrc/tfrg_dense.hip

```cpp
#include <hip/hip_runtime.h>

#include "tfrg_dense.h"
#include "tfrg_dev.h"
#include "tfrg_internal.h"

namespace tfrg {
namespace {

typedef uint32_t dn_u32x4 __attribute__((ext_vector_type(4)));
typedef uint64_t dn_u64x2 __attribute__((ext_vector_type(2)));

struct Tally {
  uint32_t trunc = 0, pad = 0, zero = 0, multi = 0, skip = 0;
};

typedef const __attribute__((address_space(4))) DenseArgs* KArgs;
typedef const __attribute__((address_space(4))) DenseSpec* KSpec;

struct Sp {
  KArgs a;
  KSpec s;
  const uint32_t* rs;
  uint64_t base;
  uint32_t W;
// ... 58 lines not shown
  }
}

template <uint32_t DT>
struct ValT {
  using type = uint32_t;
};
template <>
struct ValT<kDenseI64> {
  using type = uint64_t;
};

template <uint32_t DT>
__device__ __forceinline__ typename ValT<DT>::type value_at(const Sp& x, uint64_t e, uint32_t c, uint32_t j) {
  using T = typename ValT<DT>::type;
  const bool ok = j < c;
  const uint64_t i = ok ? e + j : 0ull;
  const T v = DT == kDenseF32 ? (T)x.a->f32[i] : (T)(uint64_t)x.a->i64[i];
  return ok ? v : (T)x.s->fill;
}

template <uint32_t DT, int K, bool ROWS>
__device__ __forceinline__ uint32_t values_from(const Sp& x, Tally& t, uint32_t r, uint32_t j,
                                                typename ValT<DT>::type* v) {
  if constexpr (!ROWS) {
    uint64_t e;
    uint32_t c;
    row_of(x, r, e, c);
#pragma unroll
    for (int k = 0; k < K; ++k) {
      if (j == 0) note_row<false>(x, t, r, 1u, c, c);
      v[k] = value_at<DT>(x, e, c, j);
      if (++j == x.W) {
        j = 0;
        ++r;
        if (k + 1 < K) row_of(x, r, e, c);
      }
    }
    return (1u << K) - 1u;
  } else {
    uint32_t rr[K], jj[K], c[K];
    uint64_t e[K];
    Rec q[K];
#pragma unroll
    for (int k = 0; k < K; ++k) {
      rr[k] = r;
      jj[k] = j;
      const bool wrap = ++j == x.W;
      r += wrap;
      j = wrap ? 0u : j;
    }
#pragma unroll
    for (int k = 0; k < K; ++k) q[k] = rec_of<true>(x, rr[k]);
#pragma unroll
    for (int k = 0; k < K; ++k) row_of(x, q[k], e[k], c[k]);
#pragma unroll
    for (int k = 0; k < K; ++k) v[k] = value_at<DT>(x, e[k], c[k], jj[k]);
    uint32_t okm = 0u;
#pragma unroll
    for (int k = 0; k < K; ++k) {
      okm |= q[k].ok << k;
      if (jj[k] == 0) note_row<true>(x, t, rr[k], q[k].ok, c[k], c[k]);
    }
    return okm;
  }
}

struct BRow {
  uint32_t off, len, cnt;
};

__device__ __forceinline__ BRow brow_of(const Sp& x, const Rec& q) {
  uint64_t e;
  uint32_t c;
  row_of(x, q, e, c);
  const uint64_t es = c ? e : 0ull;
  BRow b{0u, 0u, c};
  if (x.a->b_off64) {
    const uint64_t o0 = x.a->b_off64[es], o1 = x.a->b_off64[es + 1];
    const uint64_t l = o1 - o0;
    b.off = o0 < 0xffffffffull ? (uint32_t)o0 : 0xffffffffu;
    b.len = l < 0xffffffffull ? (uint32_t)l : 0xffffffffu;
  } else {
    b.off = x.a->b_off[es];
    b.len = x.s->const_len != kDenseNoLen ? x.s->const_len : x.a->b_len[es];
  }
  if (!c) b.len = 0u;
  return b;
}

template <bool ROWS>
__device__ __forceinline__ BRow brow_of(const Sp& x, uint32_t r, uint32_t& ok) {
  const Rec q = rec_of<ROWS>(x, r);
  ok = q.ok;
  return brow_of(x, q);
}

template <bool ROWS>
__device__ __forceinline__ void note_brow(const Sp& x, Tally& t, uint32_t r, uint32_t ok, const BRow& b) {
  note_row<ROWS>(x, t, r, ok, b.cnt, b.len);
  t.multi += b.cnt > 1u;
}

__device__ __forceinline__ uint32_t in_byte(const Sp& x, const BRow& b, uint32_t j) {
  const uint64_t p = (uint64_t)b.off + j;
  if (p >= x.a->in_bound) return 0u;
  return (uint32_t)__builtin_amdgcn_raw_buffer_load_b8(x.in, (uint32_t)p, 0, 0);
}

template <int K, bool ROWS>
__device__ __forceinline__ uint32_t u8_dwords4(const Sp& x, Tally& t, uint32_t r, uint32_t j, uint32_t* w) {
  uint32_t rr[K], jj[K];
  BRow bb[K];
  Rec q[K];
#pragma unroll
  for (int k = 0; k < K; ++k) {
    rr[k] = r;
    jj[k] = j;
    j += 4u;
    const bool wrap = j == x.W;
    r += wrap;
    j = wrap ? 0u : j;
  }
#pragma unroll
  for (int k = 0; k < K; ++k) q[k] = rec_of<ROWS>(x, rr[k]);
#pragma unroll
  for (int k = 0; k < K; ++k) bb[k] = brow_of(x, q[k]);
  uint32_t d0[K], d1[K];
#pragma unroll
  for (int k = 0; k < K; ++k) {
    const uint64_t p = (uint64_t)bb[k].off + jj[k];
    const bool ok = bb[k].len > jj[k] && p < x.a->in_bound;
    const uint32_t p0 = ok ? ((uint32_t)p & ~3u) : 0xfffffff8u;
    d0[k] = (uint32_t)__builtin_amdgcn_raw_buffer_load_b32(x.in, p0, 0, 0);
    d1[k] = (uint32_t)__builtin_amdgcn_raw_buffer_load_b32(x.in, p0 + 4u, 0, 0);
  }
  const uint32_t fill = ((uint32_t)x.s->fill & 0xffu) * 0x01010101u;
#pragma unroll
  for (int k = 0; k < K; ++k) {
    const uint32_t left = bb[k].len > jj[k] ? bb[k].len - jj[k] : 0u;
    const uint32_t m = left >= 4u ? 0xffffffffu : (1u << (8u * left)) - 1u;
    const uint32_t d = __builtin_amdgcn_alignbyte(d1[k], d0[k], (bb[k].off + jj[k]) & 3u);
    w[k] = (d & m) | (fill & ~m);
  }
  uint32_t okm = 0u;
#pragma unroll
  for (int k = 0; k < K; ++k) {
    okm |= q[k].ok << k;
    if (jj[k] == 0) note_brow<ROWS>(x, t, rr[k], q[k].ok, bb[k]);
  }
  return okm;
}

template <bool ROWS>
__device__ __forceinline__ uint32_t u8_dword(const Sp& x, Tally& t, uint32_t& r, uint32_t& j, BRow& b, uint32_t& ok,
                                             bool more, uint32_t& okm) {
  const uint32_t fill = (uint32_t)x.s->fill & 0xffu;
  uint32_t w = 0u;
  okm = 0u;
#pragma unroll
  for (int k = 0; k < 4; ++k) {
    if (j == 0) note_brow<ROWS>(x, t, r, ok, b);
    w |= (j < b.len ? in_byte(x, b, j) : fill) << (8 * k);
    okm |= ok << k;
    if (++j == x.W) {
      j = 0;
      ++r;
// ... 226 lines not shown
```

### tfrecords-reader_amd/csrc/tfrg_internal.h

```cpp
#pragma once
#include <stdint.h>
#include <hip/hip_runtime.h>
#include "tfrg_layout.h"

namespace tfrg {

struct DevSchema {
  uint32_t n_keys;
  uint32_t n_slots;
  uint32_t ht_mask;
  const uint32_t* ht;
  const uint32_t* key_hash;
  const uint32_t* key_off;
  const uint8_t* key_blob;
  const int32_t* key_slot;
  const uint8_t* slot_kind;
  const uint32_t* key_w;
  const uint32_t* krec;
  const uint32_t* tpl;
  const uint32_t* tpl_img;
  uint32_t tpl_img_words;
  uint32_t tpl_tab_words;
  uint32_t n_tpl;
  uint32_t tpl_w;
  const uint32_t* spec;
};

constexpr uint32_t kCrcTabWords = 51200;

struct LeanTgt {
  uint16_t* ord;
  uint32_t* cnt;
  uint2* loc;
  uint32_t* rs;
  void* v1;
  uint32_t* v2;
  uint32_t lim;
  uint32_t kind;
  uint32_t pad[2];
};
struct LeanArgs {
  uint32_t n_tpl;
  uint32_t lane_max;
  uint32_t* tsum;
  uint32_t n_slots;
  uint32_t tile_stride;
  uint32_t img_words;
  uint32_t gpw;
  uint32_t bsplit;
  uint32_t gsplit;
  const uint8_t* finish;
  uint32_t implicit;
  uint32_t tab_words;
  uint32_t cu_lds;
  uint32_t stage_any;
  uint32_t gpw_force;
  uint32_t nocrc;
  uint32_t strict;
  uint32_t uframes;
  LeanTgt tg[kLeanMaxSlots];
};

enum KeyRec : uint32_t { kKrHash = 0, kKrLen, kKrW0, kKrW1, kKrSlot1, kKrSlot2, kKrSlot3, kKrFlags, kKrWords };
constexpr uint32_t kLdsMaxKeys = 256;
constexpr uint32_t kLdsMaxHt = 1024;
inline bool schema_in_lds(const DevSchema& sc) { return sc.n_keys <= kLdsMaxKeys && sc.ht_mask + 1 <= kLdsMaxHt; }

__host__ __device__ inline uint32_t key_hash_words(uint32_t n, uint32_t w0, uint32_t w1) {
  const uint32_t a = (w0 ^ (w0 >> 11) ^ (n << 17)) & 0xffffffu;
  const uint32_t b = (w1 ^ (w1 >> 13) ^ (n << 7)) & 0xffffffu;
#if defined(__HIP_DEVICE_COMPILE__)
  uint32_t p0, p1;
  asm("v_mul_u32_u24 %0, %1, %2" : "=v"(p0) : "v"(a), "v"(0x9E3779u));
  asm("v_mul_u32_u24 %0, %1, %2" : "=v"(p1) : "v"(b), "v"(0x85EBCBu));
  uint32_t h = p0 ^ p1;
#else
  uint32_t h = a * 0x9E3779u;
  h ^= b * 0x85EBCBu;
#endif
  return h ^ (h >> 15);
}

enum OffMode : uint32_t { kOffU64 = 0, kOffU32 = 1, kOffEnds = 2 };

struct DevBatch {
  const uint8_t* bytes;
  uint64_t nbytes;
  const uint64_t* start;
  const uint64_t* end;
  const uint32_t* start32;
  const uint32_t* end32;
  uint32_t first;
  uint32_t omode;
  uint32_t n;
  uint32_t flags;
};

#if defined(__HIPCC__)
__device__ __forceinline__ uint64_t rec_end(const DevBatch& B, uint32_t r) {
  return B.omode == kOffU64 ? B.end[r] : (uint64_t)B.end32[r];
}
__device__ __forceinline__ uint64_t rec_start(const DevBatch& B, uint32_t r) {
  if (B.omode == kOffU64) return B.start[r];
  if (B.omode == kOffU32) return B.start32[r];
  return r ? (uint64_t)B.end32[r - 1] : (uint64_t)B.first;
}
#endif

enum InfoIdx : uint32_t {
  kInfoErrors = 0,
  kInfoFirstError = 1,
  kInfoMissRecords = 2,
  kInfoMissEntries = 3,
  kInfoBig = 4,
  kInfoScanTimeout = 5,
  kInfoHuge = 6,
  kInfoSlow = 7,
  kInfoSpineDone = 8,
  kInfoNeed = 9,
  kInfoSpineTicket = 10,
  kInfoOverflow = 11,
  kInfoBytesTicket = 12,
// ... 30 lines not shown
  uint32_t* rs;
  uint64_t* slot_base;
  uint32_t* totals;
  uint64_t* kind_totals;
  int64_t* i64;
  uint32_t* f32;
  uint32_t* b_off;
  uint32_t* b_len;
  uint64_t cap_i64, cap_f32, cap_b;
  uint32_t* big_list;
  uint32_t* miss;
  uint32_t miss_cap;
  uint32_t* info;
  uint32_t* info_next;
  uint32_t* tsum;
  uint32_t tile_stride;
  uint64_t* spine_lb;
  uint32_t n_chunks;
  uint32_t* slow_list;
  uint32_t* crc_rec;
  uint64_t* crc_base;
  uint64_t* crc_part;
  uint32_t* irr;
  uint4* dq;
  uint8_t* dq_cnt;
  uint32_t dq_blocks;
  uint64_t* lmask;
  uint32_t* rlist;
};

constexpr uint32_t kTileShift = 8;
constexpr uint32_t kTileRecs = 1u << kTileShift;
constexpr uint32_t kSpineChunkShift = 12;

constexpr uint32_t kFlagPayloadOnly = 1u;
constexpr uint32_t kFlagSpecVarint = 2u;
constexpr uint32_t kFlagNoCrc = 4u;
constexpr uint32_t kFlagStrictCrc = 8u;
constexpr uint32_t kFlagMaterializeBytes = 16u;


struct DevBytes {
  const uint8_t* in;
  uint64_t in_readable;
  const uint32_t* b_off;
  const uint32_t* b_len;
  const uint64_t* kind_totals;
  uint64_t* offsets;
  uint64_t offsets_cap;
  uint8_t* data;
  uint64_t data_cap;
  uint64_t* lb;
  uint32_t* ticket;
  uint32_t* big_count;
  uint32_t* big_list;
  uint32_t* overflow;
};
hipError_t launch_materialize(const DevBytes& d, int num_cus, hipStream_t st);
uint64_t materialize_lb_words(uint64_t cap_b);

struct LaunchCfg {
  int num_cus;
  bool lean;
  bool tpl_full;
  bool tpl_unchecked;
  const uint32_t* spec_h;
  int lane_grid;
  int wave_grid;
  uint32_t lane_max;
  uint32_t wave_stage;
  bool body_count;
  uint32_t poison[4];
  bool optimistic;
  bool ran_optimistic;
  bool ord_const;
  bool len_const;
  bool ran_quiet_big;
  uint32_t tpl_cu_lds;
  bool tpl_stage_any;
  uint32_t tpl_gpw;
  bool walk_beside;
  uint32_t walk_blocks;
  uint32_t implicit;
};

enum Stage : int { kStageTplLane = 0, kStageLaneCount, kStageBodyCount, kStageTailCount, kStageSpine,
                   kStageDownGather, kStageTailGather, kStageMaterialize, kNumStages };
extern const char* const kStageNames[kNumStages];

hipError_t launch_tpl_lane(const DevBatch& b, const DevOut& o, const LeanArgs& a, const uint32_t* img, uint32_t w,
                           int num_cus, hipStream_t st);
int lane_count_mode(const DevSchema& sc);
void launch_lane_count(const DevBatch& b, const DevSchema& sc, const DevOut& o, const uint32_t* d_tab,
                       const LaunchCfg& cfg, bool defer_big, int mode, int max_blocks, hipStream_t st);
void launch_body_count(const DevBatch& b, const DevOut& o, int num_cus, hipStream_t st);
bool tail_walk_fits(const DevSchema& sc);
void launch_tail_count(const DevBatch& b, const DevSchema& sc, const DevOut& o, const uint32_t* d_tab,
                       const uint32_t* d_consts, const LaunchCfg& cfg, bool finish, bool walk, uint32_t max_blocks,
                       hipStream_t st);
void launch_poison_loc(const DevOut& o, uint32_t n, uint32_t n_slots, const uint32_t recs[4], hipStream_t st);
void launch_spine(const DevOut& o, const DevSchema& sc, uint32_t n_tiles, uint32_t n, hipStream_t st);
void launch_down_gather(const DevBatch& b, const DevSchema& sc, const DevOut& o, const LaunchCfg& cfg,
                        uint32_t n_tiles, uint32_t resident, hipStream_t st);
void launch_tail_gather(const DevBatch& b, const DevSchema& sc, const DevOut& o, const LaunchCfg& cfg, int max_blocks,
                        hipStream_t st);
hipError_t launch_fill_placed_rows(uint32_t* rs, const uint32_t* info, uint32_t n_slots, uint32_t n, hipStream_t st);
hipError_t launch_stream_read(const void* d, uint64_t nbytes, uint32_t* sink, hipStream_t st, int variant);
struct FrTab;
hipError_t launch_frame_index(const FrTab& T, int num_cus, hipStream_t st);
hipError_t launch_decode(const DevBatch& b, const DevSchema& sc, const DevOut& o, LaunchCfg& cfg,
                         const uint32_t* d_crc_tables, const uint32_t* d_wave_consts, hipStream_t stream,
                         hipEvent_t* ev);

}
```

### tfrecords-reader_amd/csrc/tfrg_learn.cpp

```cpp
#include "tfrg_learn.h"

#include <string.h>

#include <algorithm>
#include <map>

#include "../../include/tfrg.h"
#include "crc32c.h"
#include "tfrg_layout.h"

namespace tfrg {

static_assert(TFRG_TPL_MAX == kTplMaxLane && TFRG_TPL_MAX_PAYLOAD == kTplMaxL && TFRG_TPL_MAX_ENTRIES == kTplMaxEntries &&
                  TFRG_TPL_MAX_SLOTS == kLeanMaxSlots && TFRG_TPL_SAMPLE == kTplSample,
              "tfrg.h mirrors tfrg_layout.h");

namespace {


const CrcTables& crc_tables() {
  static const CrcTables T = [] {
    CrcTables t;
    crc_make_tables(&t);
    return t;
// ... 256 lines not shown
    d[kLtAbsent] = ~present & (S >= kLeanMaxSlots ? 0xffffu : ((1u << S) - 1u));
  }
  const uint32_t tw = kLiTw(W);
  std::vector<uint32_t> img(kLiTpl + (size_t)nt * tw, 0);
  img[0] = nt;
  img[1] = W;
  img[2] = tw;
  img[4] = W;
  std::vector<uint8_t> lut(kTplMaxL + 1, 0xffu);
  for (uint32_t k = 0; k < nt; ++k) {
    const uint32_t* d = &w[(size_t)k * kLtWords];
    uint32_t* q = &img[kLiTpl + (size_t)k * tw];
    const uint32_t L = d[kLtL];
    q[0] = L;
    q[1] = d[kLtK];
    q[2] = 0xffu;
    q[3] = d[kLtFrame];
    for (uint32_t i = 0; i < 3 * W; ++i) q[4 + i] = d[kLtWin + (i / W) * W + i % W];
    for (uint32_t s2 = 0; s2 < kLeanMaxSlots; ++s2) {
      const uint32_t* z = d + kLtSlot + 3 * s2;
      uint32_t* y = q + 4 + 3 * W + 4 * s2;
      y[0] = z[0];
      y[1] = z[1];
      y[2] = z[2];
      const uint32_t mode = z[0] & 0xffu, rk = z[0] >> 16;
      uint32_t& sq = img[kLiSlotQ + s2];
      if (rk && (mode == 1u || mode == 2u)) {
        const uint32_t qw = z[1] >> 2;
        const uint32_t lo = (sq & kLiQValue) ? std::min(sq & 0xffu, qw) : qw;
        const uint32_t hi = (sq & kLiQValue) ? std::max((sq >> 8) & 0xffu, qw) : qw;
        sq = (sq & kLiQSingle) | kLiQValue | lo | (hi << 8);
      }
      if (k == 0) sq |= kLiQSingle;
      if ((z[2] & ~kCountInline) > 1u) sq &= ~kLiQSingle;
    }
    img[3] |= d[kLtCrcw];
    img[4] = std::min(img[4], d[kLtChain]);
    if (lut[L] == 0xffu) {
      lut[L] = (uint8_t)k;
    } else {
      uint32_t p = lut[L];
      while (img[kLiTpl + (size_t)p * tw + 2] != 0xffu) p = img[kLiTpl + (size_t)p * tw + 2];
      img[kLiTpl + (size_t)p * tw + 2] = k;
    }
  }
  memcpy(&img[kLiLut], lut.data(), lut.size());
  {
    const uint32_t used = (img[3] & 0xffu) | (img[4] < W ? 0x80u : 0u);
    uint32_t np = 0;
    for (uint32_t j = 0; j < 8; ++j) {
      if (!(used & (1u << j))) continue;
      img[6 + j / 4] |= np << (8 * (j % 4));
      out.ptab.resize((size_t)(np + 1) * kLiPtabWords);
      uint32_t* t = &out.ptab[(size_t)np * kLiPtabWords];
      for (uint32_t v = 0; v < 256; ++v) {
        uint32_t x = CT.t[0][v];
        for (uint32_t d = 0; d < 32; ++d) {
          if (d >= 28 - 4 * j && d < 32 - 4 * j) t[(d - (28 - 4 * j)) * 256 + v] = x;
          x = (x >> 8) ^ CT.t[0][x & 0xff];
        }
      }
      ++np;
    }
    img[5] = np;
  }
  out.ord_const = S > 0 && S <= kLeanMaxSlots;
  for (uint32_t s2 = 0; out.ord_const && s2 < S; ++s2) {
    const uint32_t r0 = w[kLtSlot + 3 * s2] >> 16;
    out.ord_const = r0 != 0;
    for (uint32_t k = 1; out.ord_const && k < nt; ++k) out.ord_const = (w[(size_t)k * kLtWords + kLtSlot + 3 * s2] >> 16) == r0;
  }
  out.len_const = S > 0 && S <= kLeanMaxSlots;
  out.const_len.assign(S, 0u);
  for (uint32_t s2 = 0; out.len_const && s2 < S; ++s2) {
    if ((c->slot_kind[s2] & 3u) != TFRG_KIND_BYTES) continue;
    const uint32_t z0 = w[kLtSlot + 3 * s2];
    out.len_const = (z0 & 0xffu) == 3u && (z0 >> 16) != 0;
    for (uint32_t k = 1; out.len_const && k < nt; ++k) {
      const uint32_t zk = w[(size_t)k * kLtWords + kLtSlot + 3 * s2];
      out.len_const = (zk & 0xffu) == 3u && (zk >> 16) != 0 && ((zk >> 8) & 0xffu) == ((z0 >> 8) & 0xffu);
    }
    out.const_len[s2] = (z0 >> 8) & 0xffu;
  }
  out.w = std::move(w);
  out.spec = std::move(spec);
  out.img = std::move(img);
  out.img.resize((out.img.size() + 3) & ~(size_t)3, 0u);
  out.W = W;
  out.have_spec = have_spec;
  return nt;
}

bool learn_single_slots(const TplSchema* c, uint32_t S, const uint8_t* h_bytes, uint64_t nbytes,
                        const uint64_t* h_start, const uint64_t* h_end, uint32_t n, uint32_t flags,
                        std::vector<uint32_t>& spec) {
  spec.assign(S ? S : 1, 0u);
  if (!S || !n) return false;
  tfrg_host_ctx* hc = nullptr;
  if (tfrg_host_ctx_create(&hc)) return false;
  std::vector<uint32_t> single(S, 0u);
  uint32_t m = 0;
  const uint32_t lim = n < kTplSample ? n : kTplSample;
  for (uint32_t j = 0; j < lim; ++j) {
    const uint32_t i = (uint32_t)((uint64_t)j * n / lim);
    uint64_t a = h_start[i], e = h_end[i];
    if (e > nbytes || e < a) continue;
    if (!(flags & TFRG_FLAG_PAYLOAD_ONLY)) {
      if (e - a < 16) continue;
      a += 12;
      e -= 4;
    }
    tfrg_host_record rec;
    if (tfrg_host_decode(hc, h_bytes + a, e - a, flags, &rec) || rec.status != TFRG_OK) continue;
    ++m;
    for (uint32_t k = 0; k < rec.n_entries; ++k) {
      const auto it = c->key_id.find(std::string((const char*)h_bytes + a + rec.key_off[k], rec.key_len[k]));
      if (it == c->key_id.end()) continue;
      const uint32_t kind = rec.kind[k];
      if (kind < 1 || kind > 3) continue;
      const int32_t slot = c->key_slot[4ull * it->second + kind];
      if (slot < 0 || (uint32_t)slot >= S || rec.val_cnt[k] != 1) continue;
      if (kind == TFRG_KIND_INT64) {
        const int64_t v = rec.i64[rec.val_off[k]];
        if (v < 0 || v >= (int64_t)1 << 28) continue;
      }
      ++single[slot];
    }
  }
  tfrg_host_ctx_destroy(hc);
  if (!m) return false;
  return place_single_slots(c, S, single, m, spec);
}

}

using namespace tfrg;

extern "C" int tfrg_learn_templates_host(uint32_t n_keys, const uint8_t* key_blob, const uint64_t* key_offsets,
                                         const uint32_t* key_flags, uint32_t n_slots, const uint32_t* slot_key,
                                         const uint8_t* slot_kind, const uint8_t* h_bytes, uint64_t nbytes,
                                         const uint64_t* h_start, const uint64_t* h_end, uint32_t n, uint32_t flags,
                                         uint32_t* out, uint64_t cap, uint32_t* window_words) {
  if (n && (!h_bytes || !h_start || !h_end)) return TFRG_E_ARG;
  std::unordered_map<std::string, uint32_t> key_id;
  std::vector<int32_t> ks(4ull * (n_keys ? n_keys : 1), -1);
  for (uint32_t k = 0; k < n_keys; ++k) {
    key_id.emplace(std::string((const char*)key_blob + key_offsets[k], key_offsets[k + 1] - key_offsets[k]), k);
    ks[4ull * k] = (int32_t)(key_flags ? (key_flags[k] & 1u) : 0u);
  }
  for (uint32_t s2 = 0; s2 < n_slots; ++s2) {
    if (slot_key[s2] >= n_keys || slot_kind[s2] < 1 || slot_kind[s2] > 3) return TFRG_E_ARG;
    ks[4ull * slot_key[s2] + slot_kind[s2]] = (int32_t)s2;
  }
  std::vector<uint8_t> sk(slot_kind, slot_kind + n_slots);
  const TplSchema sch{key_id, ks, sk};
  Learned L;
  const uint32_t nt = learn_shapes(&sch, n_slots, h_bytes, nbytes, h_start, h_end, n, flags, L);
  if (window_words) *window_words = L.W;
  if (out && nt) memcpy(out, L.w.data(), std::min<uint64_t>(L.w.size(), cap) * 4);
  return (int)nt;
}
```

### tfrecords-reader_amd/csrc/tfrg_learn.h

```cpp
#pragma once
#include <stdint.h>

#include <string>
#include <unordered_map>
#include <vector>

namespace tfrg {

struct TplSchema {
  const std::unordered_map<std::string, uint32_t>& key_id;
  const std::vector<int32_t>& key_slot;
  const std::vector<uint8_t>& slot_kind;
};

struct Learned {
  std::vector<uint32_t> w, spec, img;
  std::vector<uint32_t> ptab;
  uint32_t W = 0;
  bool have_spec = false;
  bool full = false;
  uint32_t frames = 0;
  bool ord_const = false;
  bool len_const = false;
  std::vector<uint32_t> const_len;
};

uint32_t learn_shapes(const TplSchema* c, uint32_t S, const uint8_t* h_bytes, uint64_t nbytes, const uint64_t* h_start,
                      const uint64_t* h_end, uint32_t n, uint32_t flags, Learned& out);

bool learn_single_slots(const TplSchema* c, uint32_t S, const uint8_t* h_bytes, uint64_t nbytes,
                        const uint64_t* h_start, const uint64_t* h_end, uint32_t n, uint32_t flags,
                        std::vector<uint32_t>& spec);

}
```

### tfrecords-reader_amd/csrc/tfrg_ragged.h

```cpp
#pragma once
#include <stdint.h>
#include <hip/hip_runtime.h>

namespace tfrg {

constexpr uint32_t kRaggedMaxSpecs = 64;
constexpr uint32_t kRaggedTileMin = 64, kRaggedTileMax = 4096, kRaggedTileDefault = 1024;
constexpr uint32_t kRaggedScanThreads = 1024;
constexpr uint32_t kRaggedChunk = 1024;
constexpr uint32_t kRaggedMaxSplit = 256;
constexpr uint32_t kRaggedNoLen = 0xffffffffu;

struct RaggedSpec {
  void* values;
  int64_t* offsets;
  uint64_t cap;
  uint32_t slot;
  uint32_t dtype;
  uint32_t max_len;
  uint32_t const_len;
};

struct RaggedArgs {
  const uint32_t* rs;
  const uint64_t* slot_base;
  const int64_t* i64;
  const uint32_t* f32;
  const uint32_t* b_off;
  const uint32_t* b_len;
  const uint64_t* b_off64;
  const uint8_t* in;
  const uint32_t* info;
  uint32_t* stats;
  uint64_t* totals;
  uint64_t* tsum;
  const void* rows;
  int64_t row0;
  uint32_t m;
  uint32_t rows64;
  uint32_t in_bound;
  uint32_t n;
  uint32_t n_specs;
  uint32_t tile;
  uint32_t tiles;
  uint32_t split;
  RaggedSpec sp[kRaggedMaxSpecs];
};
static_assert(sizeof(RaggedArgs) <= 4096, "the spec table travels as the kernel argument");

hipError_t launch_ragged(const RaggedArgs& a, hipStream_t st);

}
```

### tfrecords-reader_amd/csrc/tfrg_ragged.hip

```cpp
#include <hip/hip_runtime.h>

#include "tfrg_dense.h"
#include "tfrg_dev.h"
#include "tfrg_internal.h"
#include "tfrg_ragged.h"

namespace tfrg {
namespace {

typedef uint32_t rg_u32x4 __attribute__((ext_vector_type(4)));
typedef uint64_t rg_u64x2 __attribute__((ext_vector_type(2)));

constexpr uint32_t kBlk = 256;

typedef const __attribute__((address_space(4))) RaggedArgs* KArgs;
typedef const __attribute__((address_space(4))) RaggedSpec* KSpec;

struct Sp {
  KArgs a;
  KSpec s;
  const uint32_t* rs;
  uint64_t base;
  uint32_t max_len;
  __amdgpu_buffer_rsrc_t in;
  const uint8_t* rows;
  int64_t row0;
  uint32_t rsh, rhi;
};

__device__ __forceinline__ Sp make_sp(KArgs a, uint32_t si) {
  const KSpec s = &a->sp[si];
  const uint32_t* const info = a->info;
  const uint64_t placed = ((uint64_t)info[kInfoPlacedHi] << 32) | info[kInfoPlacedLo];
  const uint32_t slot = s->slot;
  Sp x;
  x.a = a;
  x.s = s;
  x.base = a->slot_base[slot];
  x.rs = (slot < 64u && ((placed >> slot) & 1ull)) ? nullptr : a->rs + (uint64_t)slot * ((uint64_t)a->n + 1u);
  x.max_len = s->max_len;
  x.in = __builtin_amdgcn_make_buffer_rsrc(const_cast<uint8_t*>(a->in), (short)0, (int)a->in_bound, 0x00020000);
  x.rows = static_cast<const uint8_t*>(a->rows);
  x.row0 = a->row0;
  x.rsh = a->rows64 ? 3u : 2u;
  x.rhi = a->rows64 ? 4u : 0u;
  return x;
}

struct Rec {
  uint32_t g;
  uint32_t ok;
};

__device__ __forceinline__ Rec rec_of(const Sp& x, uint32_t k) {
  int64_t v = (int64_t)k;
  if (x.rows) {
    const uint8_t* const p = x.rows + ((uint64_t)k << x.rsh);
    const uint32_t lo = *reinterpret_cast<const uint32_t*>(p);
    const uint32_t hi = *reinterpret_cast<const uint32_t*>(p + x.rhi);
    v = x.rhi ? (int64_t)(((uint64_t)hi << 32) | lo) : (int64_t)(int32_t)lo;
  }
  const uint64_t d = (uint64_t)v - (uint64_t)x.row0;
  const bool ok = v >= x.row0 && d < (uint64_t)x.a->n;
  uint32_t okv = ok ? 1u : 0u;
  asm("" : "+v"(okv));
  return Rec{ok ? (uint32_t)d : 0u, okv};
}

struct Row {
  uint32_t len;
  uint32_t L;
  uint32_t cnt;
  uint32_t src;
  uint32_t ok;
};

template <bool U8>
__device__ __forceinline__ Row row_of(const Sp& x, uint32_t k) {
  const Rec q = rec_of(x, k);
  uint32_t lo = q.g, c = 1u;
  if (x.rs) {
    lo = x.rs[q.g];
    c = x.rs[q.g + 1u] - lo;
  }
  c = q.ok ? c : 0u;
  Row r;
  r.ok = q.ok;
  r.cnt = c;
  if constexpr (!U8) {
    r.src = lo;
    r.L = c;
  } else {
    const uint64_t es = c ? x.base + lo : 0ull;
    uint32_t off, len;
    if (x.a->b_off64) {
      const uint64_t o0 = x.a->b_off64[es], o1 = x.a->b_off64[es + 1];
      const uint64_t l = o1 - o0;
      off = o0 < 0xffffffffull ? (uint32_t)o0 : 0xffffffffu;
      len = l < 0xffffffffull ? (uint32_t)l : 0xffffffffu;
    } else {
      off = x.a->b_off[es];
      len = x.s->const_len != kRaggedNoLen ? x.s->const_len : x.a->b_len[es];
    }
    r.src = off;
    r.L = c ? len : 0u;
  }
  r.len = (x.max_len && r.L > x.max_len) ? x.max_len : r.L;
  return r;
}

__device__ __forceinline__ uint32_t wave_sum(uint32_t v) {
#pragma unroll
  for (int d = 32; d >= 1; d >>= 1) v += __shfl_down(v, d, 64);
  return v;
}

__device__ __forceinline__ uint64_t wave_sum64(uint64_t v) {
#pragma unroll
  for (int d = 32; d >= 1; d >>= 1) v += (uint64_t)__shfl_down((unsigned long long)v, d, 64);
  return v;
}

__device__ __forceinline__ uint64_t wave_incl_scan64(uint64_t v) {
  const uint32_t lane = threadIdx.x & 63u;
#pragma unroll
  for (int o = 1; o < 64; o <<= 1) {
    const uint64_t u = (uint64_t)__shfl_up((unsigned long long)v, o, 64);
    if (lane >= (uint32_t)o) v += u;
  }
  return v;
}

template <int W>
__device__ __forceinline__ uint64_t block_excl_scan64(uint64_t v, uint64_t* part, uint64_t* total) {
  const uint64_t inc = wave_incl_scan64(v);
  const uint32_t w = threadIdx.x >> 6;
  __syncthreads();
  if ((threadIdx.x & 63u) == 63u) part[w] = inc;
  __syncthreads();
  uint64_t before = 0, all = 0;
#pragma unroll
  for (int i = 0; i < W; ++i) {
    const uint64_t s = part[i];
    before += (uint32_t)i < w ? s : 0ull;
    all += s;
  }
  *total = all;
  return before + inc - v;
}

template <bool U8>
__device__ __forceinline__ uint64_t len_tile(const Sp& x, uint32_t t0, uint32_t t1, uint32_t& trunc, uint32_t& empty,
                                             uint32_t& multi, uint32_t& skip) {
  uint64_t sum = 0;
  for (uint32_t k = t0 + threadIdx.x; k < t1; k += kBlk) {
    const Row r = row_of<U8>(x, k);
    sum += r.len;
    trunc += r.L > r.len;
    empty += r.ok & (uint32_t)(r.cnt == 0u);
    if constexpr (U8) multi += r.cnt > 1u;
    skip += r.ok ^ 1u;
  }
  return sum;
}

__global__ __launch_bounds__(kBlk) void k_rg_len(const RaggedArgs) {
  __shared__ uint64_t part[kBlk / 64];
  const KArgs a = (KArgs)__builtin_amdgcn_kernarg_segment_ptr();
  const uint32_t tiles = a->tiles;
  const uint32_t si = blockIdx.x / tiles, ti = blockIdx.x - si * tiles;
  const Sp x = make_sp(a, si);
  const uint32_t t0 = ti * a->tile;
  const uint32_t t1 = a->m - t0 < a->tile ? a->m : t0 + a->tile;
  uint32_t trunc = 0, empty = 0, multi = 0, skip = 0;
  uint64_t sum;
  if (x.s->dtype == kDenseU8) sum = len_tile<true>(x, t0, t1, trunc, empty, multi, skip);
  else sum = len_tile<false>(x, t0, t1, trunc, empty, multi, skip);
  sum = wave_sum64(sum);
  if ((threadIdx.x & 63u) == 0u) part[threadIdx.x >> 6] = sum;
  __syncthreads();
  if (threadIdx.x == 0) {
    uint64_t all = 0;
#pragma unroll
    for (uint32_t i = 0; i < kBlk / 64; ++i) all += part[i];
// ... 234 lines not shown
```

### tfrecords-reader_amd/csrc/tfrg_scan.hip

```cpp
#include <algorithm>
#include "tfrg_dev.h"

namespace tfrg {

constexpr int kSpineBlock = 256;
constexpr int kSpineItems = 16;
static_assert(kSpineBlock * kSpineItems == (1 << kSpineChunkShift), "one chunk per spine workgroup");

__device__ __forceinline__ uint32_t spine_look_back(const uint64_t* lb, uint32_t chunk, uint32_t lane) {
  uint32_t excl = 0;
  for (int64_t base = (int64_t)chunk - 1; base >= 0;) {
    const int64_t j = base - (int64_t)lane;
    const uint64_t w = j >= 0 ? __hip_atomic_load(&lb[j], __ATOMIC_RELAXED, __HIP_MEMORY_SCOPE_AGENT)
                              : (2ull << 32);
    const uint32_t flag = (uint32_t)(w >> 32);
    const uint64_t inc = __ballot(flag == 2u), unset = __ballot(flag == 0u);
    const uint32_t stop = inc ? (uint32_t)__builtin_ctzll(inc) : 64u;
    const uint64_t range = stop >= 63u ? ~0ull : (2ull << stop) - 1ull;
    if (unset & range) {
      __builtin_amdgcn_s_sleep(1);
      continue;
    }
    uint32_t v = lane <= stop ? (uint32_t)w : 0u;
#pragma unroll
// ... 235 lines not shown
        if (k >= S) break;
        if (sk[g]) continue;
        const uint32_t kind = sc.slot_kind[k];
        const uint64_t sbase = o.slot_base[k];
  #pragma unroll
        for (uint32_t t = 0; t < kDT; ++t) {
          if (tile0 + t >= n_tiles) break;
          uint32_t pre = o.tsum[(size_t)k * o.tile_stride + tile0 + t];
          for (uint32_t w = 0; w < wib; ++w) pre += s_w[buf][t * kDG + g][w];
          const uint32_t rsv = pre + ex[t][g];
          if (valid[t]) o.rs[(size_t)k * (B.n + 1) + r[t]] = rsv;
          if (c[t][g] & kCountInline) put_inline(o, kind, lc[t][g], sbase + rsv);
          else if (c[t][g]) need |= 1u << t;
        }
      }
      buf ^= 1u;
    }
  #pragma unroll
    for (uint32_t t = 0; t < kDT; ++t) {
      const bool nd = (need >> t) & 1u;
      const uint64_t nm = __ballot(nd);
      if (nm) {
        const int f = __builtin_ctzll(nm);
        uint32_t b0 = 0;
        if (lane == (uint32_t)f) b0 = atomicAdd(&o.info[kInfoNeed], (uint32_t)__popcll(nm));
        b0 = __shfl(b0, f, 64);
        if (nd) o.slow_list[b0 + (uint32_t)__popcll(nm & ((1ull << lane) - 1ull))] = r[t];
      }
    }
    __syncthreads();
    const uint32_t t_end = tile0 + kDT < n_tiles ? tile0 + kDT : (tile0 < n_tiles ? o.tile_stride : tile0);
    const uint32_t span = t_end - tile0;
    for (uint32_t i = threadIdx.x; i < S * span; i += kLaneBlock)
      o.tsum[(size_t)(i / span) * o.tile_stride + tile0 + i % span] = 0u;
  }
  if (blockIdx.x == 0)
    for (uint32_t i = threadIdx.x; i < 2u * S * o.n_chunks; i += kLaneBlock) reinterpret_cast<uint32_t*>(o.spine_lb)[i] = 0u;
}

__global__ void k_poison_loc(DevOut o, uint32_t n, uint32_t n_slots, uint4 recs) {
  const uint32_t rr[4] = {recs.x, recs.y, recs.z, recs.w};
  for (uint32_t k = threadIdx.x; k < n_slots; k += blockDim.x)
    for (int i = 0; i < 4; ++i)
      if (rr[i] < n) o.loc[(size_t)k * n + rr[i]] = make_uint2(0xfffff000u, 0x00ffffffu);
}

void launch_poison_loc(const DevOut& o, uint32_t n, uint32_t n_slots, const uint32_t recs[4], hipStream_t st) {
  hipLaunchKernelGGL(k_poison_loc, dim3(1), dim3(64), 0, st, o, n, n_slots, make_uint4(recs[0], recs[1], recs[2], recs[3]));
}

void launch_spine(const DevOut& o, const DevSchema& sc, uint32_t n_tiles, uint32_t n, hipStream_t st) {
  hipLaunchKernelGGL(k_spine, dim3(o.n_chunks * sc.n_slots), dim3(kSpineBlock), 0, st, o, sc.slot_kind, sc.n_slots,
                     n_tiles, sc.spec, n);
}

void launch_down_gather(const DevBatch& b, const DevSchema& sc, const DevOut& o, const LaunchCfg& cfg,
                        uint32_t n_tiles, uint32_t resident, hipStream_t st) {
  const bool compat = !(b.flags & kFlagSpecVarint);
  const bool four = n_tiles >= 16u * (uint32_t)cfg.num_cus;
  const uint32_t ng = four ? (n_tiles + 3) / 4 : n_tiles;
  const auto fn = four ? (compat ? &k_down_gather<true, 4> : &k_down_gather<false, 4>)
                       : (compat ? &k_down_gather<true, 1> : &k_down_gather<false, 1>);
  hipLaunchKernelGGL(fn, dim3(ng < resident ? ng : resident), dim3(kLaneBlock), 0, st, b, sc, o, cfg.lane_max, n_tiles);
}

__global__ __launch_bounds__(256) void k_fill_placed_rows(uint32_t* __restrict__ rs, const uint32_t* __restrict__ info,
                                                          uint32_t n_slots, uint32_t n) {
  const uint64_t placed = ((uint64_t)info[kInfoPlacedHi] << 32) | info[kInfoPlacedLo];
  const uint32_t k = blockIdx.y;
  if (k >= 64u || k >= n_slots || !((placed >> k) & 1ull)) return;
  uint32_t* row = rs + (size_t)k * (n + 1u);
  for (uint32_t i = blockIdx.x * 256u + threadIdx.x; i <= n; i += gridDim.x * 256u) row[i] = i;
}

hipError_t launch_fill_placed_rows(uint32_t* rs, const uint32_t* info, uint32_t n_slots, uint32_t n, hipStream_t st) {
  const uint32_t slots = n_slots < 64u ? n_slots : 64u;
  if (!slots) return hipSuccess;
  const uint32_t blocks = (n + 1u + 255u) / 256u;
  hipLaunchKernelGGL(k_fill_placed_rows, dim3(blocks < 1024u ? blocks : 1024u, slots), dim3(256), 0, st, rs, info,
                     n_slots, n);
  return hipGetLastError();
}

}
```

### tfrecords-reader_amd/csrc/tfrg_tpl.hip

```cpp
#include <hip/hip_runtime.h>
#include "tfrg_internal.h"
#include "tfrg_dev.h"
#include "crc32c.h"
#include "../../include/tfrg_status.h"

namespace tfrg {

namespace {

constexpr int kTplBlock = 512;
constexpr uint32_t kTplTabWords = 8;
static_assert(4u * kTplTabWords * kLiPtabWords + 4u * kLiMaxWords + 512u <= 65536u, "lane image + CRC tables exceed LDS");
constexpr uint32_t kStageWords = 1024 + 32, kStageRounds = (kStageWords * 4u + 1023u) / 1024u;
constexpr uint32_t kStTimgWords = (53248u - 64u - (kTplBlock / 64u) * kStageWords * 4u) / 16u * 4u;
template <bool ST>
__device__ __forceinline__ uint32_t* st_timg() {
  if constexpr (ST) {
    __shared__ __attribute__((aligned(16))) uint32_t s_timg[kStTimgWords];
    return s_timg;
  } else {
    return nullptr;
  }
}
template <bool ST>
// ... 204 lines not shown
    const bool valid = r < B.n;
    const uint32_t st = start_of(f), en = f.e;
    const bool inb = in_batch(g, st, en);
    const uint32_t rl = en - st;
    uint32_t cand = inb && rl >= 16u && rl - 16u <= kTplMaxL && rl <= A.lane_max ? (uint32_t)lut[rl - 16u] : 0xffu;
    uint32_t tsel = 0xffu;
    while (__ballot(cand != 0xffu)) {
      const bool act = cand != 0xffu;
      const uint32_t* tp = limg + kLiTpl + (act ? cand : 0u) * kTw;
      const u32x4 meta = *reinterpret_cast<const u32x4*>(tp);
      uint32_t diff = 0;
#pragma unroll
      for (int q = 0; q < W / 4; ++q) {
        const u32x4 bm = *reinterpret_cast<const u32x4*>(tp + 4 + 4 * q);
        const u32x4 mm = *reinterpret_cast<const u32x4*>(tp + 4 + W + 4 * q);
        diff |= ((w[4 * q] ^ bm.x) & mm.x) | ((w[4 * q + 1] ^ bm.y) & mm.y) | ((w[4 * q + 2] ^ bm.z) & mm.z) |
                ((w[4 * q + 3] ^ bm.w) & mm.w);
        if (q & 1) __builtin_amdgcn_sched_barrier(0);
      }
      const uint32_t* cm = tp + 4 + 2 * W;
      uint32_t c = 0;
      if (chain_u < (uint32_t)(W - 9)) {
#pragma unroll
        for (int i = 0; i < W - 9; ++i)
          if ((uint32_t)i >= chain_u) c = lin_word(tabw(7), c ^ (w[i] & cm[i]));
      }
      uint32_t lin = 0;
#define TFRG_LIN(j)                                                                                       \
  if (crcw_u & (1u << (j))) lin ^= lin_word(tabw(j), (w[W - 9 + (j)] & cm[W - 9 + (j)]) ^ ((j) == 0 ? c : 0u));
      TFRG_LIN(0) TFRG_LIN(1) TFRG_LIN(2) TFRG_LIN(3) TFRG_LIN(4) TFRG_LIN(5) TFRG_LIN(6) TFRG_LIN(7)
#undef TFRG_LIN
      bool ok = act && diff == 0u;
      if constexpr (UF) {
        const uint32_t mc = crc_mask(lin ^ meta.y);
        ok = ok && (nocrc || (meta.w ? mc != 0u && !A.strict : mc == w[W - 1]));
      } else {
        ok = ok && crc_mask(lin ^ meta.y) == w[W - 1];
      }
      tsel = ok ? cand : tsel;
      cand = act && !ok ? meta.z : 0xffu;
    }
    const bool hit = tsel != 0xffu;
    if (hit && !(A.implicit & TFRG_IMPLICIT_STATUS)) {
      o.status[r] = TFRG_OK;
      if constexpr (UF)
        o.verdict[r] = (uint8_t)(nocrc || limg[kLiTpl + tsel * kTw + 3] ? (uint32_t)TFRG_V_LEN_MATCH : kHitVerdict);
      else
        o.verdict[r] = (uint8_t)kHitVerdict;
    }
    if (__ballot(hit)) {
      const uint32_t* ts = limg + kLiTpl + (hit ? tsel : 0u) * kTw + 4 + 3 * W;
      for (uint32_t k = 0; k < A.n_slots; ++k) {
        const uint32_t sq = gimg[kLiSlotQ + k];
        const u32x4 z = *reinterpret_cast<const u32x4*>(ts + 4u * k);
        const uint32_t mode = z.x & 0xffu, len = (z.x >> 8) & 0xffu, pos = z.y, cw = z.z;
        uint32_t lx = pos, ly = len;
        if (sq & kLiQValue) {
          const uint32_t qw = pos >> 2;
          uint32_t a = 0, b = 0;
          for (uint32_t i = sq & 0xffu; i <= ((sq >> 8) & 0xffu); ++i) {
            const bool at = qw == i;
            a = at ? wsel(w, i) : a;
            b = at ? wsel(w, i + 1u) : b;
          }
          const uint32_t x = __builtin_amdgcn_alignbyte(b, a, pos & 3u);
          if (mode == 1u || mode == 2u) {
            lx = mode == 1u ? vgroups(x, bytes_mask(len)) : x;
            ly = 0;
          }
        }
        if (mode == 3u) lx = en + pos;
        const uint32_t tot = !A.tsum ? 0u
                             : (sq & kLiQSingle) ? (uint32_t)__popcll(__ballot(hit && cw != 0u))
                                                 : wave_sum(hit ? (cw & ~kCountInline) : 0u);
        const LeanTgt& T = A.tg[k];
        if (hit) {
          if (!(A.implicit & TFRG_IMPLICIT_ORDER)) T.ord[r] = (uint16_t)(z.x >> 16);
          if (T.kind) {
            if (r < T.lim) {
              constexpr bool kNt = ST && TFRG_TPL_STORE_NT;
              if (T.kind == TFRG_KIND_INT64) {
                st_nt<kNt>(reinterpret_cast<uint64_t*>(T.v1) + r, (uint64_t)lx);
              } else {
                st_nt<kNt>(reinterpret_cast<uint32_t*>(T.v1) + r, lx);
                if (T.kind == TFRG_KIND_BYTES && !(A.implicit & TFRG_IMPLICIT_BYTES_LEN)) st_nt<kNt>(T.v2 + r, ly);
              }
            }
          } else {
            T.cnt[r] = cw;
            T.loc[r] = make_uint2(lx, ly);
          }
        }
        acc += lane == k ? tot : 0u;
      }
    }
    const uint64_t mm = __ballot(valid && !hit);
    if (lane == 0) {
      o.lmask[g] = mm;
      if (mm) o.rlist[atomicAdd(&o.info[kInfoResid], 1u)] = g;
    }
    listed += mm ? 1u : 0u;
  };
  auto flush = [&](uint32_t g) {
    if (lane < A.n_slots && acc && A.tsum) {
      if (whole)
        A.tsum[lane * A.tile_stride + (g >> 2)] = acc;
      else
        atomicAdd(&A.tsum[lane * A.tile_stride + (g >> 2)], acc);
    }
    acc = 0;
  };
  LaneOff fa = offsets(gbeg), f0 = offsets(gbeg + 1u);
  static_assert(kTplTabWords * kLiPtabWords % (4u * kTplBlock) == 0u, "table copy in whole 16-byte rounds");
  constexpr uint32_t kTabRounds = kTplTabWords * kLiPtabWords / (4u * kTplBlock);
  const uint32_t tab16 = A.tab_words >> 2;
  u32x4 tv[kTabRounds];
#pragma unroll
  for (uint32_t j = 0; j < kTabRounds; ++j)
    if (threadIdx.x + j * kTplBlock < tab16) tv[j] = reinterpret_cast<const u32x4*>(tabs)[threadIdx.x + j * kTplBlock];
  const uint32_t iw0 = threadIdx.x < A.img_words ? img[threadIdx.x] : 0u;
  wvec wa;
  Span sa{0u, false};
  if constexpr (ST)
    sa = fill(fa, gbeg);
  else
    window(wa, fa);
#pragma unroll
  for (uint32_t j = 0; j < kTabRounds; ++j)
    if (threadIdx.x + j * kTplBlock < tab16) reinterpret_cast<u32x4*>(tab)[threadIdx.x + j * kTplBlock] = tv[j];
  if (threadIdx.x < A.img_words) limg[threadIdx.x] = iw0;
  for (uint32_t i = threadIdx.x + kTplBlock; i < A.img_words; i += kTplBlock) limg[i] = img[i];
  __syncthreads();
  if constexpr (ST) {
    for (uint32_t g = gbeg; g < gend; ++g) {
      asm volatile("" ::: "memory");
      __builtin_amdgcn_s_waitcnt(0x0F70);
      asm volatile("" ::: "memory");
      take(wa, fa, g, sa);
      asm volatile("" ::: "memory");
      __builtin_amdgcn_s_waitcnt(0xC07F);
      asm volatile("" ::: "memory");
      Span sn{0u, false};
      if (g + 1u < gend) sn = fill(f0, g + 1u);
      const LaneOff f2 = offsets(g + 2u);
      head_fix(wa, fa, g);
      proc(wa, g, fa);
      if (((g + 1u) & 3u) == 0u || g + 1u >= gend) flush(g);
      fa = f0;
      f0 = f2;
      sa = sn;
    }
  } else {
    for (uint32_t g = gbeg; g < gend; ++g) {
      head_fix(wa, fa, g);
      proc(wa, g, fa);
      if (((g + 1u) & 3u) == 0u || g + 1u >= gend) flush(g);
      if (g + 1u < gend) {
        window(wa, f0);
        fa = f0;
        f0 = offsets(g + 2u);
      }
    }
  }
  if (A.finish) {
    __shared__ uint32_t s_listed[kWaves];
    __shared__ uint32_t s_last, s_total;
    if (lane == 0) s_listed[wib] = listed;
// ... 81 lines not shown
```

### tfrecords-reader_amd/tfr_reader/_native.py

```python

from __future__ import annotations

import ctypes as C
import os
from pathlib import Path

_LIB: C.CDLL | None = None
_LIB_PATH = Path(os.environ.get("TFRG_LIB", Path(__file__).with_name("libtfrg.so")))

u8p = C.POINTER(C.c_uint8)
u16p = C.POINTER(C.c_uint16)
u32p = C.POINTER(C.c_uint32)
u64p = C.POINTER(C.c_uint64)
i32p = C.POINTER(C.c_int32)
i64p = C.POINTER(C.c_int64)


class TfrgInfo(C.Structure):
    _fields_ = [
        ("n_records", C.c_uint32),
        ("n_slots", C.c_uint32),
        ("n_errors", C.c_uint32),
        ("first_error", C.c_uint32),
        ("n_miss_records", C.c_uint32),
        ("n_miss_entries", C.c_uint32),
        ("n_big", C.c_uint32),
        ("scan_timeout", C.c_uint32),
        ("kind_totals", C.c_uint64 * 4),
        ("nbytes", C.c_uint64),
        ("bytes_data_len", C.c_uint64),
        ("tpl_groups_missed", C.c_uint32),
        ("implicit_cols", C.c_uint32),
        ("placed_slots", C.c_uint64),
    ]


class TfrgHostRecord(C.Structure):
    _fields_ = [
        ("status", C.c_int32),
        ("n_entries", C.c_uint32),
        ("aux", C.c_int64),
        ("key_off", u32p),
        ("key_len", u32p),
        ("kind", u8p),
        ("val_off", u32p),
        ("val_cnt", u32p),
        ("i64", i64p),
        ("f32", u32p),
        ("b_off", u32p),
        ("b_len", u32p),
    ]


class TfrgColumns(C.Structure):
    _fields_ = [
        ("status", i32p),
        ("aux", i64p),
        ("verdict", u8p),
        ("order", u16p),
        ("row_splits", u32p),
        ("slot_base", u64p),
        ("i64", i64p),
        ("f32", u32p),
        ("bytes_off", u32p),
        ("bytes_len", u32p),
        ("miss", u32p),
        ("bytes_data", u8p),
        ("bytes_offsets", u64p),
    ]


class TfrgIndexInfo(C.Structure):
    _fields_ = [
        ("n_records", C.c_uint64),
        ("fallback", C.c_uint32),
        ("tiled", C.c_uint32),
        ("first_start", C.c_uint32),
        ("n_chunks", C.c_uint32),
        ("repaired_chunks", C.c_uint32),
        ("repair_rounds", C.c_uint32),
    ]


INDEX_FB_ROUNDS = 1
INDEX_FB_SEEK = 2


class TfrgDenseSpec(C.Structure):
    _fields_ = [
        ("slot", C.c_uint32),
        ("dtype", C.c_uint32),
        ("width", C.c_uint32),
        ("reserved", C.c_uint32),
        ("fill", C.c_uint64),
        ("out", C.c_void_p),
        ("lengths", C.c_void_p),
    ]


DENSE_I64 = 0
DENSE_I32 = 1
DENSE_F32 = 2
DENSE_U8 = 3
DENSE_MAX_SPECS = 64
DENSE_MAX_WIDTH = 4096
ROWS_I32 = 0
ROWS_I64 = 1


class TfrgRaggedSpec(C.Structure):
    _fields_ = [
        ("slot", C.c_uint32),
        ("dtype", C.c_uint32),
        ("max_len", C.c_uint32),
        ("reserved", C.c_uint32),
        ("cap", C.c_uint64),
# ... 30 lines not shown
SEL_EQ = 0
SEL_NE = 1
SEL_LT = 2
SEL_LE = 3
SEL_GT = 4
SEL_GE = 5
SEL_APPEND = 1
SEL_TILE_MIN = 64
SEL_TILE_MAX = 4096
SEL_TILE_DEFAULT = 1024
SEL_SCAN_THREADS = 1024

SIGNATURES: dict[str, tuple] = {
    "tfrg_abi_version": (C.c_int, []),
    "tfrg_last_error": (C.c_char_p, []),
    "tfrg_status_exception": (C.c_char_p, [C.c_int]),
    "tfrg_status_message": (C.c_char_p, [C.c_int, C.c_int64]),
    "tfrg_index_buffer": (C.c_int64, [C.c_void_p, C.c_uint64, u64p, C.c_int64]),
    "tfrg_index_file": (C.c_int, [C.c_char_p, C.POINTER(u64p), i64p]),
    "tfrg_idx_save": (C.c_int, [C.c_char_p, u64p, C.c_int64]),
    "tfrg_idx_load": (C.c_int, [C.c_char_p, C.POINTER(u64p), i64p]),
    "tfrg_free": (None, [C.c_void_p]),
    "tfrg_gather_ranges": (C.c_uint64, [C.c_void_p, u64p, u64p, C.c_int64, C.c_void_p]),
    "tfrg_scan_keys": (C.c_int64, [C.c_void_p, C.c_uint64, u64p, u64p, C.c_int64, C.c_uint32, u64p, C.c_int64]),
    "tfrg_crc32c": (C.c_uint32, [C.c_void_p, C.c_uint64]),
    "tfrg_compression_of": (C.c_int, [C.c_void_p, C.c_uint64]),
    "tfrg_inflate": (C.c_int, [C.c_void_p, C.c_uint64, C.POINTER(u8p), u64p]),
    "tfrg_masked_crc32c": (C.c_uint32, [C.c_void_p, C.c_uint64]),
    "tfrg_frame_records": (C.c_int64, [C.c_void_p, u64p, C.c_int64, C.c_int, C.c_void_p, C.c_int64]),
    "tfrg_ctx_create": (C.c_int, [C.c_int, C.POINTER(C.c_void_p)]),
    "tfrg_ctx_destroy": (C.c_int, [C.c_void_p]),
    "tfrg_ctx_set_lane_max": (C.c_int, [C.c_void_p, C.c_uint32]),
    "tfrg_ctx_set_wave_stage": (C.c_int, [C.c_void_p, C.c_uint32]),
    "tfrg_ctx_set_record_bound": (C.c_int, [C.c_void_p, C.c_uint64]),
    "tfrg_learn_templates": (C.c_int, [C.c_void_p, C.c_void_p, C.c_uint64, C.c_void_p, C.c_void_p, C.c_uint32,
                                       C.c_uint32]),
    "tfrg_host_ctx_create": (C.c_int, [C.c_void_p]),
    "tfrg_host_ctx_destroy": (C.c_int, [C.c_void_p]),
    "tfrg_host_decode": (C.c_int, [C.c_void_p, C.c_char_p, C.c_uint64, C.c_uint32, C.POINTER(TfrgHostRecord)]),
    "tfrg_template_count": (C.c_int, [C.c_void_p]),
    "tfrg_template_frames": (C.c_int, [C.c_void_p]),
    "tfrg_template_words": (C.c_int, [C.c_void_p, C.c_void_p, C.c_uint64, C.c_void_p]),
    "tfrg_learn_templates_host": (C.c_int, [C.c_uint32, C.c_void_p, C.c_void_p, C.c_void_p, C.c_uint32, C.c_void_p,
                                            C.c_void_p, C.c_void_p, C.c_uint64, C.c_void_p, C.c_void_p, C.c_uint32,
                                            C.c_uint32, C.c_void_p, C.c_uint64, C.c_void_p]),
    "tfrg_ctx_set_templates": (C.c_int, [C.c_void_p, C.c_int]),
    "tfrg_stream_read": (C.c_int, [C.c_void_p, C.c_uint64, C.c_void_p, C.c_void_p, C.c_int]),
    "tfrg_device_count": (C.c_int, []),
    "tfrg_stream_create": (C.c_int, [C.c_int, C.c_uint64, C.c_int, C.POINTER(C.c_void_p)]),
    "tfrg_stream_destroy": (C.c_int, [C.c_void_p]),
    "tfrg_stream_ctx": (C.c_void_p, [C.c_void_p, C.c_int]),
    "tfrg_stream_submit": (C.c_int, [C.c_void_p, C.c_int, C.POINTER(C.c_void_p), C.POINTER(C.c_char_p), u64p, u64p,
                                     C.c_int, C.c_uint32]),
    "tfrg_stream_wait": (C.c_int, [C.c_void_p, C.c_int, u64p, u64p, u64p, C.c_int, C.POINTER(C.c_double)]),
    "tfrg_stream_host_buffer": (C.c_void_p, [C.c_void_p, C.c_int]),
    "tfrg_stream_result": (C.c_int, [C.c_void_p, C.c_int, C.POINTER(TfrgInfo), C.POINTER(TfrgColumns)]),
    "tfrg_stream_host_ranges": (C.c_int, [C.c_void_p, C.c_int, C.POINTER(u64p), C.POINTER(u64p)]),
    "tfrg_ctx_set_profiling": (C.c_int, [C.c_void_p, C.c_int]),
    "tfrg_ctx_set_value_caps": (C.c_int, [C.c_void_p, C.c_uint64, C.c_uint64, C.c_uint64]),
    "tfrg_ctx_device_bytes": (C.c_int, [C.c_void_p, C.POINTER(C.c_uint64), C.POINTER(C.c_uint64)]),
    "tfrg_profile_last": (C.c_int, [C.c_void_p, C.POINTER(C.c_float), C.POINTER(C.c_char_p), C.c_int]),
    "tfrg_set_schema": (
        C.c_int,
        [C.c_void_p, C.c_uint32, C.c_void_p, u64p, u32p, C.c_uint32, u32p, u8p],
    ),
    "tfrg_decode_device": (
        C.c_int,
        [C.c_void_p, C.c_void_p, C.c_uint64, C.c_void_p, C.c_void_p, C.c_uint32, C.c_uint32, C.c_void_p],
    ),
    "tfrg_decode_device32": (
        C.c_int,
        [C.c_void_p, C.c_void_p, C.c_uint64, C.c_void_p, C.c_void_p, C.c_uint32, C.c_uint32, C.c_uint32,
         C.c_void_p],
    ),
    "tfrg_decode_host": (
        C.c_int,
        [C.c_void_p, C.c_void_p, C.c_uint64, u64p, u64p, C.c_uint32, C.c_uint32, C.c_void_p],
    ),
    "tfrg_ctx_set_index_chunk": (C.c_int, [C.c_void_p, C.c_uint32]),
    "tfrg_index_device": (C.c_int, [C.c_void_p, C.c_void_p, C.c_uint64, u64p, C.c_uint32, C.c_void_p, C.c_void_p,
                                    C.c_void_p, C.c_uint64, u64p, C.c_void_p, C.POINTER(TfrgIndexInfo)]),
    "tfrg_stream_set_device_index": (C.c_int, [C.c_void_p, C.c_int]),
    "tfrg_result_info": (C.c_int, [C.c_void_p, C.POINTER(TfrgInfo)]),
    "tfrg_result_device": (C.c_int, [C.c_void_p, C.POINTER(TfrgColumns)]),
    "tfrg_result_fetch": (C.c_int, [C.c_void_p, C.POINTER(TfrgColumns)]),
    "tfrg_result_dense": (C.c_int, [C.c_void_p, C.POINTER(TfrgDenseSpec), C.c_uint32, C.c_void_p, C.c_void_p]),
    "tfrg_result_dense_rows": (C.c_int, [C.c_void_p, C.POINTER(TfrgDenseSpec), C.c_uint32, C.c_void_p, C.c_uint32,
                                         C.c_uint32, C.c_int64, C.c_void_p, C.c_void_p, C.c_void_p]),
    "tfrg_result_ragged_rows": (C.c_int, [C.c_void_p, C.POINTER(TfrgRaggedSpec), C.c_uint32, C.c_void_p, C.c_uint32,
                                          C.c_uint32, C.c_int64, C.c_void_p, C.c_void_p, C.c_void_p]),
    "tfrg_ctx_set_ragged_tile": (C.c_int, [C.c_void_p, C.c_uint32]),
    "tfrg_result_select_rows": (C.c_int, [C.c_void_p, C.POINTER(TfrgSelectTerm), C.c_uint32, C.c_void_p, C.c_uint32,
                                          C.c_uint32, C.c_int64, C.c_void_p, C.c_uint32, C.c_uint64, C.c_void_p,
                                          C.c_void_p, C.c_uint32, C.c_void_p]),
    "tfrg_ctx_set_select_tile": (C.c_int, [C.c_void_p, C.c_uint32]),
}

FLAG_PAYLOAD_ONLY = 1
FLAG_SPEC_VARINT = 2
FLAG_NO_CRC = 4
FLAG_STRICT_CRC = 8
FLAG_MATERIALIZE_BYTES = 16


class NativeError(RuntimeError):
    pass


def lib() -> C.CDLL:
    global _LIB
    if _LIB is None:
        if not _LIB_PATH.exists():
            raise ImportError(
                f"libtfrg.so not found at {_LIB_PATH}: build it with "
                "`make -C tfrecords-reader_amd/csrc` (or __graft_entry__.build())"
            )
        lib_ = C.CDLL(str(_LIB_PATH))
        for name, (res, args) in SIGNATURES.items():
            fn = getattr(lib_, name)
            fn.restype = res
            fn.argtypes = args
        _LIB = lib_
    return _LIB


def check(rc: int, what: str) -> None:
    if rc != 0:
        msg = lib().tfrg_last_error().decode("utf-8", "replace")
        raise NativeError(f"{what} failed ({rc}): {msg}")


def ptr(arr, ctype=C.c_void_p):
    return arr.ctypes.data_as(ctype)
```

### tfrecords-reader_amd/tfr_reader/hip.py

```python

from __future__ import annotations

import contextlib
import ctypes as C
import gc
import threading
from collections.abc import Sequence

import numpy as np

from tfr_reader import _native as N
from tfr_reader import _status as S

try:
    from tfr_reader import _tfrg_py as _PY
except ImportError:
    _PY = None

KIND_NAMES = {1: "bytes_list", 2: "float_list", 3: "int64_list"}


_GC_LOCK = threading.Lock()
_GC_DEPTH = 0
_GC_RESTORE = False


@contextlib.contextmanager
def _no_gc():
    global _GC_DEPTH, _GC_RESTORE
    with _GC_LOCK:
        if _GC_DEPTH == 0:
            _GC_RESTORE = gc.isenabled()
            gc.disable()
        _GC_DEPTH += 1
    try:
        yield
    finally:
        with _GC_LOCK:
            _GC_DEPTH -= 1
            if _GC_DEPTH == 0 and _GC_RESTORE:
                gc.enable()

DEFAULT_LANE_MAX = 2048
KIND_IDS = {v: k for k, v in KIND_NAMES.items()}


def _as_u8(buf) -> np.ndarray:
    if isinstance(buf, np.ndarray):
        return buf.reshape(-1).view(np.uint8)
    return np.frombuffer(buf, dtype=np.uint8)


class KeyTable:

    def __init__(self) -> None:
        self.key_ids: dict[bytes, int] = {}
        self.keys: list[bytes] = []
        self.key_str: list[str | None] = []
        self.slots: dict[tuple[int, int], int] = {}
        self.slot_key: list[int] = []
        self.slot_kind: list[int] = []
        self.version = 0
        self.lock = threading.RLock()

    def intern(self, key: bytes, kind: int) -> bool:
        with self.lock:
            return self._intern(key, kind)

    def _intern(self, key: bytes, kind: int) -> bool:
        new = False
        kid = self.key_ids.get(key)
        if kid is None:
            kid = len(self.keys)
            self.key_ids[key] = kid
            self.keys.append(key)
            try:
                self.key_str.append(key.decode("utf-8"))
            except UnicodeDecodeError:
                self.key_str.append(None)
            new = True
        if kind and self.key_str[kid] is not None and (kid, kind) not in self.slots:
            self.slots[(kid, kind)] = len(self.slot_key)
            self.slot_key.append(kid)
            self.slot_kind.append(kind)
            new = True
        if new:
            self.version += 1
        return new


class HipDecoder:

    def __init__(self, device: int = 0, spec_varint: bool = False, keys: KeyTable | None = None) -> None:
        self._lib = N.lib()
        self.device = device
        self.spec_varint = spec_varint
        self.keys = keys or KeyTable()
        self._pushed = -1
        self._lock = threading.Lock()
        h = C.c_void_p()
        N.check(self._lib.tfrg_ctx_create(device, C.byref(h)), "tfrg_ctx_create")
        self._ctx = h

    @classmethod
    def wrap(cls, ctx: int, device: int, keys: KeyTable, spec_varint: bool = False) -> HipDecoder:
        d = cls.__new__(cls)
        d._lib = N.lib()
        d.device = device
        d.spec_varint = spec_varint
        d.keys = keys
        d._pushed = -1
        d._lock = threading.Lock()
        d._ctx = C.c_void_p(ctx)
        d._owned = False
        return d

    def close(self) -> None:
        if self._ctx and getattr(self, "_owned", True):
            self._lib.tfrg_ctx_destroy(self._ctx)
        self._ctx = None

    def __del__(self):
        try:
            self.close()
        except Exception:
            pass

    def set_lane_max(self, nbytes: int) -> None:
        N.check(self._lib.tfrg_ctx_set_lane_max(self._ctx, nbytes), "tfrg_ctx_set_lane_max")

    def set_templates(self, on: bool) -> None:
        N.check(self._lib.tfrg_ctx_set_templates(self._ctx, int(bool(on))), "tfrg_ctx_set_templates")

    def template_count(self) -> int:
        return int(self._lib.tfrg_template_count(self._ctx))

    def template_frames(self) -> int:
        return int(self._lib.tfrg_template_frames(self._ctx))

    def learn_templates(self, buf: np.ndarray, starts: np.ndarray, ends: np.ndarray, payload_only: bool = False) -> int:
        b = np.ascontiguousarray(buf, np.uint8)
        st = np.ascontiguousarray(starts, np.uint64)
        en = np.ascontiguousarray(ends, np.uint64)
        k = self._lib.tfrg_learn_templates(self._ctx, N.ptr(b), b.size, N.ptr(st), N.ptr(en), st.size,
                                           N.FLAG_PAYLOAD_ONLY if payload_only else 0)
        N.check(min(k, 0), "tfrg_learn_templates")
        return int(k)


    def set_record_bound(self, nbytes: int) -> None:
        N.check(self._lib.tfrg_ctx_set_record_bound(self._ctx, int(nbytes)), "tfrg_ctx_set_record_bound")

    def set_wave_stage(self, nbytes: int) -> None:
        N.check(self._lib.tfrg_ctx_set_wave_stage(self._ctx, nbytes), "tfrg_ctx_set_wave_stage")

    def set_profiling(self, on: bool) -> None:
        N.check(self._lib.tfrg_ctx_set_profiling(self._ctx, int(on)), "tfrg_ctx_set_profiling")

    def profile_last(self) -> dict[str, float]:
        ms = (C.c_float * 16)()
        names = (C.c_char_p * 16)()
        k = self._lib.tfrg_profile_last(self._ctx, ms, names, 16)
        if k < 0:
            N.check(k, "tfrg_profile_last")
        return {names[i].decode(): float(ms[i]) for i in range(k)}

    def push_schema(self) -> None:
        kt = self.keys
        if self._pushed == kt.version:
            return
        with kt.lock:
            self._push_schema(kt)

    def _push_schema(self, kt: KeyTable) -> None:
        blob = b"".join(kt.keys)
        offs = np.zeros(len(kt.keys) + 1, np.uint64)
        if kt.keys:
            offs[1:] = np.cumsum([len(k) for k in kt.keys])
        flags = np.array([0 if s is not None else 1 for s in kt.key_str] or [0], np.uint32)
        blob_arr = np.frombuffer(blob or b"\0", np.uint8)
        sk = np.array(kt.slot_key or [0], np.uint32)
        sd = np.array(kt.slot_kind or [1], np.uint8)
        N.check(
            self._lib.tfrg_set_schema(
                self._ctx, len(kt.keys), N.ptr(blob_arr), N.ptr(offs, N.u64p), N.ptr(flags, N.u32p),
                len(kt.slot_key), N.ptr(sk, N.u32p), N.ptr(sd, N.u8p),
            ),
            "tfrg_set_schema",
        )
        self._pushed = kt.version
        self._pushed_slots = len(kt.slot_key)

    def _flags(self, payload_only: bool, crc: bool, strict_crc: bool = False, materialize_bytes: bool = False) -> int:
        f = 0
        if payload_only:
            f |= N.FLAG_PAYLOAD_ONLY
        if self.spec_varint:
            f |= N.FLAG_SPEC_VARINT
        if not crc:
            f |= N.FLAG_NO_CRC
        if strict_crc:
            f |= N.FLAG_STRICT_CRC
        if materialize_bytes:
# ... 111 lines not shown
            self._lib.tfrg_decode_device32(
                self._ctx, C.c_void_p(d_bytes), nbytes, C.c_void_p(d_start32) if d_start32 else None,
                C.c_void_p(d_end32), first_start, n,
                self._flags(payload_only, crc, strict_crc, materialize_bytes), C.c_void_p(stream) if stream else None,
            ),
            "tfrg_decode_device32",
        )
        self._last_n, self._last_host = n, None

    def set_index_chunk(self, nbytes: int) -> None:
        N.check(self._lib.tfrg_ctx_set_index_chunk(self._ctx, int(nbytes)), "tfrg_ctx_set_index_chunk")

    def index_device(self, d_bytes, nbytes: int | None = None, piece_sizes=None, *, stream: int | None = None):
        import torch

        nbytes = int(d_bytes.numel() if nbytes is None else nbytes)
        sizes = np.ascontiguousarray([nbytes] if piece_sizes is None else piece_sizes, dtype=np.uint64)
        dev = d_bytes.device
        info = N.TfrgIndexInfo()
        pr = np.zeros(max(sizes.size, 1), np.uint64)
        cap = nbytes // 16 + int(sizes.size) + 1
        while True:
            st = torch.empty(cap, dtype=torch.int64, device=dev)
            en = torch.empty(cap, dtype=torch.int64, device=dev)
            e32 = torch.empty(cap, dtype=torch.int32, device=dev)
            torch.cuda.current_stream(dev).synchronize()
            N.check(self._lib.tfrg_index_device(self._ctx, C.c_void_p(d_bytes.data_ptr()), nbytes,
                                                N.ptr(sizes, N.u64p), sizes.size, C.c_void_p(st.data_ptr()),
                                                C.c_void_p(en.data_ptr()), C.c_void_p(e32.data_ptr()), cap,
                                                N.ptr(pr, N.u64p), C.c_void_p(stream) if stream else None,
                                                C.byref(info)),
                    "tfrg_index_device")
            if info.fallback or info.n_records <= cap:
                break
            cap = int(info.n_records)
        cap = 0 if info.fallback else int(info.n_records)
        return DeviceIndex(info, st[:cap], en[:cap], e32[:cap], pr[: sizes.size].astype(np.int64))

    def decode_image(self, buf, piece_sizes=None, *, crc: bool = True, strict_crc: bool = False,
                     materialize_bytes: bool = False) -> BatchResult:
        import torch

        dev = torch.device("cuda", self.device)
        if isinstance(buf, torch.Tensor):
            d_all, host = buf, None
            nbytes = int(buf.numel()) - 32
            if nbytes < 0:
                raise ValueError("a device image needs 32 readable bytes past its end")
        else:
            host = _as_u8(buf)
            nbytes = int(host.size)
            pad = np.zeros(((nbytes + 15) & ~15) + 32, np.uint8)
            pad[:nbytes] = host
            d_all = torch.from_numpy(pad).to(dev)
        sizes = np.ascontiguousarray([nbytes] if piece_sizes is None else piece_sizes, dtype=np.uint64)
        if int(sizes.sum()) != nbytes:
            raise ValueError("piece_sizes do not sum to the image bytes")
        flags = self._flags(False, crc, strict_crc, materialize_bytes)
        with self._lock:
            ix = self.index_device(d_all[:nbytes] if nbytes else d_all[:0], nbytes, sizes)
            if host is None:
                host = d_all[:nbytes].cpu().numpy()
            if ix.fallback:
                from tfr_reader.cython import indexer as native

                parts, base = [], 0
                for sz in sizes.tolist():
                    parts.append(native.index_buffer(host[base : base + sz])[:, :2] + np.uint64(base))
                    base += sz
                se = np.concatenate(parts) if parts else np.zeros((0, 2), np.uint64)
                st = np.ascontiguousarray(se[:, 0], np.uint64)
                en = np.ascontiguousarray(se[:, 1], np.uint64)
                d_st = torch.from_numpy(st.view(np.int64)).to(dev)
                d_en = torch.from_numpy(en.view(np.int64)).to(dev)
                tiled = False
            else:
                st = ix.start.cpu().numpy().view(np.uint64)
                en = ix.end.cpu().numpy().view(np.uint64)
                d_st, d_en, tiled = ix.start, ix.end, bool(ix.tiled)
            n = int(st.size)
            self._seed_keys(host, st, en, flags)
            torch.cuda.current_stream(dev).synchronize()
            self.last_image_mode = "u32_ends" if tiled else "u64"
            while True:
                self.push_schema()
                if tiled:
                    rc = self._lib.tfrg_decode_device32(self._ctx, C.c_void_p(d_all.data_ptr()), nbytes, None,
                                                        C.c_void_p(ix.end32.data_ptr()), ix.first_start, n, flags,
                                                        None)
                else:
                    rc = self._lib.tfrg_decode_device(self._ctx, C.c_void_p(d_all.data_ptr()), nbytes,
                                                      C.c_void_p(d_st.data_ptr()), C.c_void_p(d_en.data_ptr()), n,
                                                      flags, None)
                N.check(rc, "tfrg_decode_device")
                info = self.info()
                if info.n_miss_records == 0:
                    break
                if not self._learn_misses(host, info) and self._pushed == self.keys.version:
                    raise N.NativeError("schema misses reported but no new key learned")
            self._last_n, self._last_host = n, (host, st, False)
            return self._fetch(host, st, en, info, False, materialize_bytes)

    def dense(self, specs, *, strict: bool = False, out=None, stream: int | None = None, rows=None):
        from tfr_reader import dense as D

        return D.decoder_dense(self, specs, strict=strict, out=out, stream=stream, rows=rows)

    def minibatches(self, specs, batch_size: int, *, seed: int = 0, drop_last: bool = False, where=None):
        from tfr_reader import dense as D

        return D.minibatches(self, specs, batch_size, seed=seed, drop_last=drop_last, where=where)

    def set_ragged_tile(self, rows: int) -> None:
        N.check(self._lib.tfrg_ctx_set_ragged_tile(self._ctx, int(rows)), "tfrg_ctx_set_ragged_tile")

    def ragged(self, specs, *, rows=None, capacity=None, out=None, stream: int | None = None):
        from tfr_reader import ragged as R

        return R.decoder_ragged(self, specs, rows=rows, capacity=capacity, out=out, stream=stream)

    def ragged_minibatches(self, specs, batch_size: int, *, seed: int = 0, drop_last: bool = False, capacity=None,
                           where=None):
        from tfr_reader import ragged as R

        return R.ragged_minibatches(self, specs, batch_size, seed=seed, drop_last=drop_last, capacity=capacity,
                                    where=where)

    def set_select_tile(self, rows: int) -> None:
        N.check(self._lib.tfrg_ctx_set_select_tile(self._ctx, int(rows)), "tfrg_ctx_set_select_tile")

    def select(self, where, *, rows=None, capacity=None, dtype: str = "int64", out=None, stream: int | None = None):
        from tfr_reader import select as S

        return S.decoder_select(self, where, rows=rows, capacity=capacity, dtype=dtype, out=out, stream=stream)

    def _fetch(self, buf, st, en, info: N.TfrgInfo, payload_only: bool, materialize: bool = False) -> BatchResult:
        n, ns = info.n_records, info.n_slots
        kt = info.kind_totals
        r = BatchResult()
        r.buf, r.starts, r.ends, r.payload_only = buf, st, en, payload_only
        r.status = np.empty(n, np.int32)
        r.aux = np.empty(n, np.int64)
        r.verdict = np.empty(n, np.uint8)
        r.order = np.empty((ns, n), np.uint16)
        r.row_splits = np.empty((ns, n + 1), np.uint32)
        r.slot_base = np.zeros(max(ns, 1), np.uint64)
        r.i64 = np.empty(kt[3], np.int64)
        r.f32 = np.empty(kt[2], np.uint32)
        r.bytes_off = np.empty(kt[1], np.uint32)
        r.bytes_len = np.empty(kt[1], np.uint32)
        names = ["status", "aux", "verdict", "order", "row_splits", "slot_base", "i64", "f32", "bytes_off",
                 "bytes_len"]
        if materialize:
            r.bytes_data = np.empty(info.bytes_data_len, np.uint8)
            r.bytes_offsets = np.empty(kt[1] + 1, np.uint64)
            names += ["bytes_data", "bytes_offsets"]
        cols = N.TfrgColumns()
        for name in names:
            arr = getattr(r, name)
            setattr(cols, name, N.ptr(arr, dict(N.TfrgColumns._fields_)[name]))
        N.check(self._lib.tfrg_result_fetch(self._ctx, C.byref(cols)), "tfrg_result_fetch")
        r.slot_key = [self.keys.key_str[k] for k in self.keys.slot_key[:ns]]
        r.slot_kind = list(self.keys.slot_kind[:ns])
        r.info = info
        return r

# ... 497 lines not shown
```

Baseline: 4421 GiB/s.

## Derive bytes offsets from record ends instead of storing them per row

During template learning, bytes slots whose value offset sits at a constant delta from the record end across all templates are flagged. The lean decode path then skips writing the per-row bytes_off column for those slots. Dense and ragged consumers rebuild the offset as end32[row] + delta, and a fill kernel materialises the column lazily when raw columns are requested. This removes one 4-byte store stream per bytes slot from the hot decode kernel, at the cost of extra bookkeeping and a deferred fill on the column-fetch paths.

```diff
diff --git a/include/tfrg.h b/include/tfrg.h
--- a/include/tfrg.h
+++ b/include/tfrg.h
@@ -136,7 +136,10 @@
   uint32_t tpl_groups_missed;
   uint32_t implicit_cols;
   uint64_t placed_slots;
+  uint64_t implicit_off_slots;
 } tfrg_info;
+
+int tfrg_ctx_rel_off(const tfrg_ctx* ctx, uint32_t slot, int32_t* delta);
 
 int tfrg_result_info(tfrg_ctx* ctx, tfrg_info* info);
 
diff --git a/tfrecords-reader_amd/csrc/tfrg_capi.cpp b/tfrecords-reader_amd/csrc/tfrg_capi.cpp
--- a/tfrecords-reader_amd/csrc/tfrg_capi.cpp
+++ b/tfrecords-reader_amd/csrc/tfrg_capi.cpp
@@ -142,6 +142,12 @@
   bool ord_const = false;
   bool len_const = false;
   std::vector<uint32_t> const_len;
+  bool implicit_off_on = true;
+  uint64_t off_rel = 0;
+  std::vector<int32_t> rel_off;
+  uint64_t last_off_mask = 0;
+  std::vector<int32_t> last_rel_off;
+  bool off_complete = false;
   uint32_t last_implicit = 0;
   bool last_aux_zero = false;
   uint32_t* info_pin = nullptr;
@@ -188,6 +194,7 @@
     if (v == 2 || v == 4 || v == 8) c->tpl_gpw = (uint32_t)v;
   }
   if (const char* e = getenv("TFRG_OPTIMISTIC")) c->optimistic_on = atoi(e) != 0;
+  if (const char* e = getenv("TFRG_IMPLICIT_OFF")) c->implicit_off_on = atoi(e) != 0;
   if (const char* e = getenv("TFRG_WALK_BESIDE")) c->walk_beside = atoi(e) != 0;
   if (const char* e = getenv("TFRG_WALK_BLOCKS")) c->walk_blocks = (uint32_t)atoi(e);
   if (const char* e = getenv("TFRG_DENSE_NT")) c->dense_nt = atoi(e) != 0;
@@ -521,6 +528,8 @@
   c->key_slot_h = ks;
   c->slot_kind_h.assign(slot_kind, slot_kind + n_slots);
   c->n_tpl = 0;
+  c->off_rel = 0;
+  c->rel_off.clear();
   c->tpl_learned = false;
   c->have_spec = false;
   return 0;
@@ -556,6 +565,8 @@
   c->n_tpl = 0;
   c->tpl_frames = 0;
   c->have_spec = false;
+  c->off_rel = 0;
+  c->rel_off.clear();
   if (!c->n_keys) return 0;
   const TplSchema sch{c->key_id, c->key_slot_h, c->slot_kind_h};
   Learned L;
@@ -587,6 +598,8 @@
     c->ord_const = L.ord_const;
     c->len_const = L.len_const;
     c->const_len = L.const_len;
+    c->off_rel = L.off_rel;
+    c->rel_off = L.rel_off;
   }
   if (L.have_spec) HIP_TRY(hipMemcpy(c->spec.p, L.spec.data(), spec_bytes, hipMemcpyHostToDevice));
   c->spec_h = L.spec;
@@ -816,6 +829,8 @@
   cfg.ord_const = c->ord_const;
   cfg.len_const = c->len_const && !mat;
   cfg.implicit = 0;
+  cfg.off_rel = c->implicit_off_on ? c->off_rel : 0ull;
+  cfg.implicit_off = 0;
   const uint64_t bound = c->call_bound ? c->call_bound : c->record_bound;
   c->call_bound = 0;
   c->last = tfrg_ctx::LastCall{d_bytes, nbytes, cap_in, bound, n, flags, st};
@@ -874,6 +889,9 @@
   if (n != 0 && cfg.ran_quiet_big) c->tsum_dirty = true;
   c->mat_pending = c->opt_pending && mat && S;
   c->last_implicit = n != 0 ? cfg.implicit : 0u;
+  c->last_off_mask = n != 0 ? cfg.implicit_off : 0ull;
+  if (c->last_off_mask) c->last_rel_off = c->rel_off;
+  c->off_complete = false;
   c->last_aux_zero = n != 0 && cfg.ran_optimistic && !cfg.ran_quiet_big && !(cfg.implicit & TFRG_IMPLICIT_STATUS);
   c->cols_complete = false;
   return 0;
@@ -992,7 +1010,14 @@
   info->tpl_groups_missed = h[kInfoResid];
   info->placed_slots = ((uint64_t)h[kInfoPlacedHi] << 32) | h[kInfoPlacedLo];
   info->implicit_cols = c->last_implicit;
+  info->implicit_off_slots = c->last_off_mask;
   return overflow_status(h);
+}
+
+int tfrg_ctx_rel_off(const tfrg_ctx* c, uint32_t slot, int32_t* delta) {
+  if (!c || !delta || slot >= 64u || !((c->off_rel >> slot) & 1ull) || slot >= c->rel_off.size()) return TFRG_E_ARG;
+  *delta = c->rel_off[slot];
+  return 0;
 }
 
 static std::vector<std::pair<uint64_t, uint32_t>> implicit_len_runs(const tfrg_ctx* c) {
@@ -1004,6 +1029,29 @@
     base += c->n;
   }
   return out;
+}
+
+static std::vector<std::pair<uint64_t, uint32_t>> implicit_off_runs(const tfrg_ctx* c) {
+  std::vector<std::pair<uint64_t, uint32_t>> out;
+  uint64_t base = 0;
+  for (uint32_t k = 0; k < c->n_slots; ++k) {
+    if ((c->slot_kind_h[k] & 3u) != TFRG_KIND_BYTES) continue;
+    if (k < 64u && ((c->last_off_mask >> k) & 1ull)) out.push_back({base, (uint32_t)c->last_rel_off[k]});
+    base += c->n;
+  }
+  return out;
+}
+
+static int fill_implicit_off(tfrg_ctx* c) {
+  if (!c->last_off_mask || c->off_complete || !c->n) return 0;
+  HIP_TRY(hipSetDevice(c->device));
+  for (const auto& [base, delta] : implicit_off_runs(c)) {
+    if (base >= c->cap_b) continue;
+    const uint32_t rows = (uint32_t)std::min<uint64_t>(c->n, c->cap_b - base);
+    HIP_TRY(launch_fill_rel_off(c->b_off.as<uint32_t>() + base, c->last_off.e32, delta, rows, c->last_stream));
+  }
+  c->off_complete = true;
+  return 0;
 }
 
 int tfrg_result_device(tfrg_ctx* c, tfrg_columns* d) {
@@ -1034,6 +1082,7 @@
                                   c->last_stream));
   }
   c->cols_complete = true;
+  if (const int rc = fill_implicit_off(c)) return rc;
   d->status = c->status.as<int32_t>();
   d->aux = c->aux.as<int64_t>();
   d->verdict = c->verdict.as<uint8_t>();
@@ -1107,7 +1156,14 @@
   a.in = c->materialized ? c->bdata.as<uint8_t>() : c->last.d_bytes;
   const uint64_t bound = c->materialized ? (uint64_t)c->bdata.cap & ~15ull : (c->last.nbytes + 15ull) & ~15ull;
   a.in_bound = a.in ? (uint32_t)std::min<uint64_t>(bound, 0xfffffff0ull) : 0;
-}
+  a.end32 = c->last_off_mask ? c->last_off.e32 : nullptr;
+}
+}
+
+static_assert(kDenseOffStored == kRaggedOffStored, "one const_off lookup serves both");
+static int32_t const_off_of(const tfrg_ctx* c, uint32_t slot, bool reads_off) {
+  if (!reads_off || slot >= 64u || !((c->last_off_mask >> slot) & 1ull)) return kDenseOffStored;
+  return c->last_rel_off[slot];
 }
 
 static_assert(kDenseNoLen == kRaggedNoLen && kRaggedNoLen == kSelNoLen, "one const_len lookup serves all three");
@@ -1193,6 +1249,7 @@
     d.dtype = s.dtype;
     d.width = s.width;
     d.const_len = const_len_of(c, s.slot, s.dtype == TFRG_DENSE_U8);
+    d.const_off = const_off_of(c, s.slot, s.dtype == TFRG_DENSE_U8);
     const uint64_t isz = s.dtype == TFRG_DENSE_I64 ? 8 : s.dtype == TFRG_DENSE_U8 ? 1 : 4;
     const uint64_t total = (uint64_t)out_rows * s.width * isz;
     const uint64_t work = ((uintptr_t)s.out & 15u) ? total / isz : (total >> 4) + 16;
@@ -1290,6 +1347,7 @@
       d.dtype = s.dtype;
       d.max_len = s.max_len;
       d.const_len = const_len_of(c, s.slot, s.dtype == TFRG_DENSE_U8);
+      d.const_off = const_off_of(c, s.slot, s.dtype == TFRG_DENSE_U8);
     }
     HIP_TRY(launch_ragged(a, st));
   } else {
@@ -1449,6 +1507,8 @@
   auto cl = [](uint64_t v, uint64_t cap) { return v < cap ? v : cap; };
   HIP_TRY(cp(h->i64, c->i64.p, cl(info.kind_totals[TFRG_KIND_INT64], c->cap_i64) * 8));
   HIP_TRY(cp(h->f32, c->f32.p, cl(info.kind_totals[TFRG_KIND_FLOAT], c->cap_f32) * 4));
+  if (h->bytes_off)
+    if (const int rc2 = fill_implicit_off(c)) return rc2;
   HIP_TRY(cp(h->bytes_off, c->b_off.p, cl(info.kind_totals[TFRG_KIND_BYTES], c->cap_b) * 4));
   if ((info.implicit_cols & TFRG_IMPLICIT_BYTES_LEN) && h->bytes_len) {
     for (const auto& [base, len] : implicit_len_runs(c)) std::fill_n(h->bytes_len + base, n, len);
diff --git a/tfrecords-reader_amd/csrc/tfrg_decode.cpp b/tfrecords-reader_amd/csrc/tfrg_decode.cpp
--- a/tfrecords-reader_amd/csrc/tfrg_decode.cpp
+++ b/tfrecords-reader_amd/csrc/tfrg_decode.cpp
@@ -45,6 +45,7 @@
     else if (kind == TFRG_KIND_FLOAT) t.v1 = o.f32 + base;
     else t.v1 = o.b_off + base;
     t.v2 = o.b_len + base;
+    t.no_off = kind == TFRG_KIND_BYTES && k < 64u && ((cfg.implicit_off >> k) & 1ull) ? 1u : 0u;
   }
   return a;
 }
@@ -81,6 +82,7 @@
                                                   (cfg.ord_const ? TFRG_IMPLICIT_ORDER : 0u) |
                                                   (cfg.len_const ? TFRG_IMPLICIT_BYTES_LEN : 0u)
                                             : 0u;
+  cfg.implicit_off = lean && quiet_tpl && b.omode != kOffU64 && !(b.flags & kFlagMaterializeBytes) ? cfg.off_rel : 0ull;
   DevOut ox = o;
   if (!lean) {
     ox.lmask = nullptr;
diff --git a/tfrecords-reader_amd/csrc/tfrg_dense.h b/tfrecords-reader_amd/csrc/tfrg_dense.h
--- a/tfrecords-reader_amd/csrc/tfrg_dense.h
+++ b/tfrecords-reader_amd/csrc/tfrg_dense.h
@@ -8,6 +8,7 @@
 constexpr uint32_t kDenseMaxWidth = 4096;
 enum DenseType : uint32_t { kDenseI64 = 0, kDenseI32 = 1, kDenseF32 = 2, kDenseU8 = 3 };
 constexpr uint32_t kDenseNoLen = 0xffffffffu;
+constexpr int32_t kDenseOffStored = 0x7fffffff;
 
 constexpr uint32_t kDenseChunk = 1024;
 
@@ -21,6 +22,7 @@
   uint32_t const_len;
   uint32_t blk0;
   uint32_t nblk;
+  int32_t const_off;
 };
 
 struct DenseArgs {
@@ -30,6 +32,7 @@
   const uint32_t* f32;
   const uint32_t* b_off;
   const uint32_t* b_len;
+  const uint32_t* end32;
   const uint64_t* b_off64;
   const uint8_t* in;
   const uint32_t* info;
diff --git a/tfrecords-reader_amd/csrc/tfrg_dense.hip b/tfrecords-reader_amd/csrc/tfrg_dense.hip
--- a/tfrecords-reader_amd/csrc/tfrg_dense.hip
+++ b/tfrecords-reader_amd/csrc/tfrg_dense.hip
@@ -164,7 +164,7 @@
     b.off = o0 < 0xffffffffull ? (uint32_t)o0 : 0xffffffffu;
     b.len = l < 0xffffffffull ? (uint32_t)l : 0xffffffffu;
   } else {
-    b.off = x.a->b_off[es];
+    b.off = x.s->const_off != kDenseOffStored ? x.a->end32[q.g] + (uint32_t)x.s->const_off : x.a->b_off[es];
     b.len = x.s->const_len != kDenseNoLen ? x.s->const_len : x.a->b_len[es];
   }
   if (!c) b.len = 0u;
diff --git a/tfrecords-reader_amd/csrc/tfrg_internal.h b/tfrecords-reader_amd/csrc/tfrg_internal.h
--- a/tfrecords-reader_amd/csrc/tfrg_internal.h
+++ b/tfrecords-reader_amd/csrc/tfrg_internal.h
@@ -37,7 +37,8 @@
   uint32_t* v2;
   uint32_t lim;
   uint32_t kind;
-  uint32_t pad[2];
+  uint32_t no_off;
+  uint32_t pad;
 };
 struct LeanArgs {
   uint32_t n_tpl;
@@ -234,6 +235,8 @@
   bool walk_beside;
   uint32_t walk_blocks;
   uint32_t implicit;
+  uint64_t off_rel;
+  uint64_t implicit_off;
 };
 
 enum Stage : int { kStageTplLane = 0, kStageLaneCount, kStageBodyCount, kStageTailCount, kStageSpine,
@@ -257,6 +260,7 @@
 void launch_tail_gather(const DevBatch& b, const DevSchema& sc, const DevOut& o, const LaunchCfg& cfg, int max_blocks,
                         hipStream_t st);
 hipError_t launch_fill_placed_rows(uint32_t* rs, const uint32_t* info, uint32_t n_slots, uint32_t n, hipStream_t st);
+hipError_t launch_fill_rel_off(uint32_t* off, const uint32_t* end32, uint32_t delta, uint32_t n, hipStream_t st);
 hipError_t launch_stream_read(const void* d, uint64_t nbytes, uint32_t* sink, hipStream_t st, int variant);
 struct FrTab;
 hipError_t launch_frame_index(const FrTab& T, int num_cus, hipStream_t st);
diff --git a/tfrecords-reader_amd/csrc/tfrg_learn.cpp b/tfrecords-reader_amd/csrc/tfrg_learn.cpp
--- a/tfrecords-reader_amd/csrc/tfrg_learn.cpp
+++ b/tfrecords-reader_amd/csrc/tfrg_learn.cpp
@@ -362,6 +362,20 @@
     }
     out.const_len[s2] = (z0 >> 8) & 0xffu;
   }
+  out.off_rel = 0;
+  out.rel_off.assign(S, 0);
+  for (uint32_t s2 = 0; s2 < S && s2 < kLeanMaxSlots && s2 < 64u; ++s2) {
+    if ((c->slot_kind[s2] & 3u) != TFRG_KIND_BYTES) continue;
+    const uint32_t z0 = w[kLtSlot + 3 * s2], p0 = w[kLtSlot + 3 * s2 + 1];
+    bool rel = (z0 & 0xffu) == 3u && (z0 >> 16) != 0;
+    for (uint32_t k = 1; rel && k < nt; ++k) {
+      const uint32_t* zk = &w[(size_t)k * kLtWords + kLtSlot + 3 * s2];
+      rel = (zk[0] & 0xffu) == 3u && (zk[0] >> 16) != 0 && zk[1] == p0;
+    }
+    if (!rel) continue;
+    out.off_rel |= 1ull << s2;
+    out.rel_off[s2] = (int32_t)p0;
+  }
   out.w = std::move(w);
   out.spec = std::move(spec);
   out.img = std::move(img);
diff --git a/tfrecords-reader_amd/csrc/tfrg_learn.h b/tfrecords-reader_amd/csrc/tfrg_learn.h
--- a/tfrecords-reader_amd/csrc/tfrg_learn.h
+++ b/tfrecords-reader_amd/csrc/tfrg_learn.h
@@ -23,6 +23,8 @@
   bool ord_const = false;
   bool len_const = false;
   std::vector<uint32_t> const_len;
+  uint64_t off_rel = 0;
+  std::vector<int32_t> rel_off;
 };
 
 uint32_t learn_shapes(const TplSchema* c, uint32_t S, const uint8_t* h_bytes, uint64_t nbytes, const uint64_t* h_start,
diff --git a/tfrecords-reader_amd/csrc/tfrg_ragged.h b/tfrecords-reader_amd/csrc/tfrg_ragged.h
--- a/tfrecords-reader_amd/csrc/tfrg_ragged.h
+++ b/tfrecords-reader_amd/csrc/tfrg_ragged.h
@@ -10,6 +10,7 @@
 constexpr uint32_t kRaggedChunk = 1024;
 constexpr uint32_t kRaggedMaxSplit = 256;
 constexpr uint32_t kRaggedNoLen = 0xffffffffu;
+constexpr int32_t kRaggedOffStored = 0x7fffffff;
 
 struct RaggedSpec {
   void* values;
@@ -19,6 +20,7 @@
   uint32_t dtype;
   uint32_t max_len;
   uint32_t const_len;
+  int32_t const_off;
 };
 
 struct RaggedArgs {
@@ -28,6 +30,7 @@
   const uint32_t* f32;
   const uint32_t* b_off;
   const uint32_t* b_len;
+  const uint32_t* end32;
   const uint64_t* b_off64;
   const uint8_t* in;
   const uint32_t* info;
diff --git a/tfrecords-reader_amd/csrc/tfrg_ragged.hip b/tfrecords-reader_amd/csrc/tfrg_ragged.hip
--- a/tfrecords-reader_amd/csrc/tfrg_ragged.hip
+++ b/tfrecords-reader_amd/csrc/tfrg_ragged.hip
@@ -99,7 +99,7 @@
       off = o0 < 0xffffffffull ? (uint32_t)o0 : 0xffffffffu;
       len = l < 0xffffffffull ? (uint32_t)l : 0xffffffffu;
     } else {
-      off = x.a->b_off[es];
+      off = x.s->const_off != kRaggedOffStored ? x.a->end32[q.g] + (uint32_t)x.s->const_off : x.a->b_off[es];
       len = x.s->const_len != kRaggedNoLen ? x.s->const_len : x.a->b_len[es];
     }
     r.src = off;
diff --git a/tfrecords-reader_amd/csrc/tfrg_scan.hip b/tfrecords-reader_amd/csrc/tfrg_scan.hip
--- a/tfrecords-reader_amd/csrc/tfrg_scan.hip
+++ b/tfrecords-reader_amd/csrc/tfrg_scan.hip
@@ -341,4 +341,16 @@
   return hipGetLastError();
 }
 
-}
+__global__ __launch_bounds__(256) void k_fill_rel_off(uint32_t* __restrict__ off, const uint32_t* __restrict__ end32,
+                                                      uint32_t delta, uint32_t n) {
+  for (uint32_t i = blockIdx.x * 256u + threadIdx.x; i < n; i += gridDim.x * 256u) off[i] = end32[i] + delta;
+}
+
+hipError_t launch_fill_rel_off(uint32_t* off, const uint32_t* end32, uint32_t delta, uint32_t n, hipStream_t st) {
+  if (!n) return hipSuccess;
+  const uint32_t blocks = (n + 255u) / 256u;
+  hipLaunchKernelGGL(k_fill_rel_off, dim3(blocks < 4096u ? blocks : 4096u), dim3(256), 0, st, off, end32, delta, n);
+  return hipGetLastError();
+}
+
+}
diff --git a/tfrecords-reader_amd/csrc/tfrg_tpl.hip b/tfrecords-reader_amd/csrc/tfrg_tpl.hip
--- a/tfrecords-reader_amd/csrc/tfrg_tpl.hip
+++ b/tfrecords-reader_amd/csrc/tfrg_tpl.hip
@@ -310,7 +310,7 @@
               if (T.kind == TFRG_KIND_INT64) {
                 st_nt<kNt>(reinterpret_cast<uint64_t*>(T.v1) + r, (uint64_t)lx);
               } else {
-                st_nt<kNt>(reinterpret_cast<uint32_t*>(T.v1) + r, lx);
+                if (!T.no_off) st_nt<kNt>(reinterpret_cast<uint32_t*>(T.v1) + r, lx);
                 if (T.kind == TFRG_KIND_BYTES && !(A.implicit & TFRG_IMPLICIT_BYTES_LEN)) st_nt<kNt>(T.v2 + r, ly);
               }
             }
diff --git a/tfrecords-reader_amd/tfr_reader/_native.py b/tfrecords-reader_amd/tfr_reader/_native.py
--- a/tfrecords-reader_amd/tfr_reader/_native.py
+++ b/tfrecords-reader_amd/tfr_reader/_native.py
@@ -32,6 +32,7 @@
         ("tpl_groups_missed", C.c_uint32),
         ("implicit_cols", C.c_uint32),
         ("placed_slots", C.c_uint64),
+        ("implicit_off_slots", C.c_uint64),
     ]
 
 
@@ -228,6 +229,7 @@
                                     C.c_void_p, C.c_uint64, u64p, C.c_void_p, C.POINTER(TfrgIndexInfo)]),
     "tfrg_stream_set_device_index": (C.c_int, [C.c_void_p, C.c_int]),
     "tfrg_result_info": (C.c_int, [C.c_void_p, C.POINTER(TfrgInfo)]),
+    "tfrg_ctx_rel_off": (C.c_int, [C.c_void_p, C.c_uint32, i32p]),
     "tfrg_result_device": (C.c_int, [C.c_void_p, C.POINTER(TfrgColumns)]),
     "tfrg_result_fetch": (C.c_int, [C.c_void_p, C.POINTER(TfrgColumns)]),
     "tfrg_result_dense": (C.c_int, [C.c_void_p, C.POINTER(TfrgDenseSpec), C.c_uint32, C.c_void_p, C.c_void_p]),
diff --git a/tfrecords-reader_amd/tfr_reader/hip.py b/tfrecords-reader_amd/tfr_reader/hip.py
--- a/tfrecords-reader_amd/tfr_reader/hip.py
+++ b/tfrecords-reader_amd/tfr_reader/hip.py
@@ -98,6 +98,7 @@
         self.keys = keys or KeyTable()
         self._pushed = -1
         self._lock = threading.Lock()
+        self._last_image = None
         h = C.c_void_p()
         N.check(self._lib.tfrg_ctx_create(device, C.byref(h)), "tfrg_ctx_create")
         self._ctx = h
@@ -111,6 +112,7 @@
         d.keys = keys
         d._pushed = -1
         d._lock = threading.Lock()
+        d._last_image = None
         d._ctx = C.c_void_p(ctx)
         d._owned = False
         return d
@@ -119,6 +121,7 @@
         if self._ctx and getattr(self, "_owned", True):
             self._lib.tfrg_ctx_destroy(self._ctx)
         self._ctx = None
+        self._last_image = None
 
     def __del__(self):
         try:
@@ -396,6 +399,7 @@
             self._seed_keys(host, st, en, flags)
             torch.cuda.current_stream(dev).synchronize()
             self.last_image_mode = "u32_ends" if tiled else "u64"
+            self._last_image = (d_all, ix)
             while True:
                 self.push_schema()
                 if tiled:
```

After: 4590 GiB/s (median of 6 runs). 3.8% higher.
